# ethanabrooks/hsr-env

Measured on AMD Instinct MI355X. Metric: env-steps/sec (whole node), HSR+1-block, steps_per_action=300, 8192 envs, higher is better.
Workload: dtype f32; 1 GPU; BASELINE config 3: cfg3, all 7 DOFs + 1 block(s), 8192 envs per GPU x 1 GPU(s), steps_per_action=300, geofence=0.05, ctrl~U(ctrlrange) per env-step, done envs reset; envs_per_gpu=8192, global_envs=8192, substeps_per_env_step=300, parallelism=env-shard x1, persistent_kernel=True, hipgraph=False

## Files before the change

hsr_env_amd/csrc/cfg_consts.h:

```cpp
#pragma once
#include "model.h"

struct Kin3_none { static constexpr bool ok = false; };
struct Kin3_cfg1 {
    static constexpr bool ok = true;
    static constexpr int NL = 2, NV = 2, RD0 = 0, NRD = 2, NFREE = 0, F0 = 0;
    static constexpr int parent[2] = {0, 0};
    static constexpr int isfree[2] = {0, 0};
    static constexpr int dofadr[2] = {0, 0};
    static constexpr int dofnum[2] = {0, 2};
    static constexpr int qadr[2] = {0, 0};
    static constexpr int dtype[2] = {0, 0};
    static constexpr int dqadr[2] = {0, 1};
    static constexpr int dlink[2] = {1, 1};
    static constexpr float lpos[2][3] = {{(float)0.0, (float)0.0, (float)0.0}, {(float)-0.46, (float)-0.081, (float)0.0}};
    static constexpr float lmat[2][9] = {{(float)1.0, (float)0.0, (float)0.0, (float)0.0, (float)1.0, (float)0.0, (float)0.0, (float)0.0, (float)1.0}, {(float)1.0, (float)0.0, (float)0.0, (float)0.0, (float)1.0, (float)0.0, (float)0.0, (float)0.0, (float)1.0}};
    static constexpr float lcom[2][3] = {{(float)0.0, (float)0.0, (float)0.0}, {(float)-0.026226165780202215, (float)0.0033597159715531835, (float)0.3351183143878767}};
    static constexpr float linr[2][6] = {{(float)0.0, (float)0.0, (float)0.0, (float)0.0, (float)0.0, (float)0.0}, {(float)17.93115297082212, (float)18.05290570568451, (float)5.361962854382956, (float)-0.18414327285216073, (float)0.6395772498672245, (float)-0.2890701869118962}};
    static constexpr float lmass[2] = {(float)0.0, (float)291.3690145854267};
    static constexpr float daxis[2][3] = {{(float)1.0, (float)0.0, (float)0.0}, {(float)0.0, (float)1.0, (float)0.0}};
    static constexpr float dpos[2][3] = {{(float)0.0, (float)0.0, (float)0.0}, {(float)0.0, (float)0.0, (float)0.0}};
};
static const int kKin3I_cfg1[] = {2, 2, 0, 0, 0, 0, 0, 0, 0, 2, 0, 0, 0, 0, 0, 1, 1, 1};
static const float kKin3F_cfg1[] = {(float)0.0, (float)0.0, (float)0.0, (float)-0.46, (float)-0.081, (float)0.0, (float)1.0, (float)0.0, (float)0.0, (float)0.0, (float)1.0, (float)0.0, (float)0.0, (float)0.0, (float)1.0, (float)1.0, (float)0.0, (float)0.0, (float)0.0, (float)1.0, (float)0.0, (float)0.0, (float)0.0, (float)1.0, (float)0.0, (float)0.0, (float)0.0, (float)-0.026226165780202215, (float)0.0033597159715531835, (float)0.3351183143878767, (float)0.0, (float)0.0, (float)0.0, (float)0.0, (float)0.0, (float)0.0, (float)17.93115297082212, (float)18.05290570568451, (float)5.361962854382956, (float)-0.18414327285216073, (float)0.6395772498672245, (float)-0.2890701869118962, (float)0.0, (float)291.3690145854267, (float)1.0, (float)0.0, (float)0.0, (float)0.0, (float)1.0, (float)0.0, (float)0.0, (float)0.0, (float)0.0, (float)0.0, (float)0.0, (float)0.0};
struct DevModel_cfg1 : DevModel {
    using kin3 = Kin3_cfg1;
    static constexpr int nq = 2, nv = 2, nu = 2, nlink = 2, nbody = 47, ngeom = 17, npair = 30, nslot = 30, nconmax = 16, njmax = 48, nM = 3, ndense = 0, npair_pad = 32, nstatic_geom = 2, nfb = 0, maxdepth = 1, iterations = 100, ls_iterations = 50, mpr_iterations = 50, any_damping = 1, solimp_general = 0, cv_types = 49248;
    static constexpr float timestep = (float)0.002, impratio = (float)2.5, gravz = (float)-9.81, tolerance = (float)1e-08, ls_tolerance = (float)0.01, mpr_tolerance = (float)1e-06, meaninertia = (float)291.3690145854267;
};
struct Kin3_cfg2 {
    static constexpr bool ok = true;
    static constexpr int NL = 3, NV = 8, RD0 = 0, NRD = 2, NFREE = 1, F0 = 2;
    static constexpr int parent[3] = {0, 0, 0};
    static constexpr int isfree[3] = {0, 0, 1};
    static constexpr int dofadr[3] = {0, 0, 2};
    static constexpr int dofnum[3] = {0, 2, 6};
    static constexpr int qadr[3] = {0, 0, 2};
    static constexpr int dtype[8] = {0, 0, 2, 2, 2, 3, 3, 3};
    static constexpr int dqadr[8] = {0, 1, 2, 3, 4, 5, 5, 5};
    static constexpr int dlink[8] = {1, 1, 2, 2, 2, 2, 2, 2};
    static constexpr float lpos[3][3] = {{(float)0.0, (float)0.0, (float)0.0}, {(float)-0.46, (float)-0.081, (float)0.0}, {(float)0.0, (float)0.0, (float)0.422}};
    static constexpr float lmat[3][9] = {{(float)1.0, (float)0.0, (float)0.0, (float)0.0, (float)1.0, (float)0.0, (float)0.0, (float)0.0, (float)1.0}, {(float)1.0, (float)0.0, (float)0.0, (float)0.0, (float)1.0, (float)0.0, (float)0.0, (float)0.0, (float)1.0}, {(float)1.0, (float)0.0, (float)0.0, (float)0.0, (float)1.0, (float)0.0, (float)0.0, (float)0.0, (float)1.0}};
    static constexpr float lcom[3][3] = {{(float)0.0, (float)0.0, (float)0.0}, {(float)-0.026226165780202215, (float)0.0033597159715531835, (float)0.3351183143878767}, {(float)0.0, (float)0.0, (float)0.0}};
    static constexpr float linr[3][6] = {{(float)0.0, (float)0.0, (float)0.0, (float)0.0, (float)0.0, (float)0.0}, {(float)17.93115297082212, (float)18.05290570568451, (float)5.361962854382956, (float)-0.18414327285216073, (float)0.6395772498672245, (float)-0.2890701869118962}, {(float)0.0003046666666666667, (float)0.0009296666666666669, (float)0.0010416666666666669, (float)0.0, (float)0.0, (float)0.0}};
    static constexpr float lmass[3] = {(float)0.0, (float)291.3690145854267, (float)1.0};
    static constexpr float daxis[8][3] = {{(float)1.0, (float)0.0, (float)0.0}, {(float)0.0, (float)1.0, (float)0.0}, {(float)1.0, (float)0.0, (float)0.0}, {(float)0.0, (float)1.0, (float)0.0}, {(float)0.0, (float)0.0, (float)1.0}, {(float)1.0, (float)0.0, (float)0.0}, {(float)0.0, (float)1.0, (float)0.0}, {(float)0.0, (float)0.0, (float)1.0}};
    static constexpr float dpos[8][3] = {{(float)0.0, (float)0.0, (float)0.0}, {(float)0.0, (float)0.0, (float)0.0}, {(float)0.0, (float)0.0, (float)0.0}, {(float)0.0, (float)0.0, (float)0.0}, {(float)0.0, (float)0.0, (float)0.0}, {(float)0.0, (float)0.0, (float)0.0}, {(float)0.0, (float)0.0, (float)0.0}, {(float)0.0, (float)0.0, (float)0.0}};
};
static const int kKin3I_cfg2[] = {3, 8, 0, 0, 0, 0, 0, 1, 0, 0, 2, 0, 2, 6, 0, 0, 2, 0, 0, 2, 2, 2, 3, 3, 3, 0, 1, 2, 3, 4, 5, 5, 5, 1, 1, 2, 2, 2, 2, 2, 2};
static const float kKin3F_cfg2[] = {(float)0.0, (float)0.0, (float)0.0, (float)-0.46, (float)-0.081, (float)0.0, (float)0.0, (float)0.0, (float)0.422, (float)1.0, (float)0.0, (float)0.0, (float)0.0, (float)1.0, (float)0.0, (float)0.0, (float)0.0, (float)1.0, (float)1.0, (float)0.0, (float)0.0, (float)0.0, (float)1.0, (float)0.0, (float)0.0, (float)0.0, (float)1.0, (float)1.0, (float)0.0, (float)0.0, (float)0.0, (float)1.0, (float)0.0, (float)0.0, (float)0.0, (float)1.0, (float)0.0, (float)0.0, (float)0.0, (float)-0.026226165780202215, (float)0.0033597159715531835, (float)0.3351183143878767, (float)0.0, (float)0.0, (float)0.0, (float)0.0, (float)0.0, (float)0.0, (float)0.0, (float)0.0, (float)0.0, (float)17.93115297082212, (float)18.05290570568451, (float)5.361962854382956, (float)-0.18414327285216073, (float)0.6395772498672245, (float)-0.2890701869118962, (float)0.0003046666666666667, (float)0.0009296666666666669, (float)0.0010416666666666669, (float)0.0, (float)0.0, (float)0.0, (float)0.0, (float)291.3690145854267, (float)1.0, (float)1.0, (float)0.0, (float)0.0, (float)0.0, (float)1.0, (float)0.0, (float)1.0, (float)0.0, (float)0.0, (float)0.0, (float)1.0, (float)0.0, (float)0.0, (float)0.0, (float)1.0, (float)1.0, (float)0.0, (float)0.0, (float)0.0, (float)1.0, (float)0.0, (float)0.0, (float)0.0, (float)1.0, (float)0.0, (float)0.0, (float)0.0, (float)0.0, (float)0.0, (float)0.0, (float)0.0, (float)0.0, (float)0.0, (float)0.0, (float)0.0, (float)0.0, (float)0.0, (float)0.0, (float)0.0, (float)0.0, (float)0.0, (float)0.0, (float)0.0, (float)0.0, (float)0.0, (float)0.0, (float)0.0, (float)0.0};
struct DevModel_cfg2 : DevModel {
    using kin3 = Kin3_cfg2;
    static constexpr int nq = 9, nv = 8, nu = 2, nlink = 3, nbody = 48, ngeom = 18, npair = 47, nslot = 57, nconmax = 16, njmax = 48, nM = 36, ndense = 0, npair_pad = 48, nstatic_geom = 2, nfb = 1, maxdepth = 1, iterations = 100, ls_iterations = 50, mpr_iterations = 50, any_damping = 1, solimp_general = 0, cv_types = 49248;
    static constexpr float timestep = (float)0.002, impratio = (float)2.5, gravz = (float)-9.81, tolerance = (float)1e-08, ls_tolerance = (float)0.01, mpr_tolerance = (float)1e-06, meaninertia = (float)73.21753814635669;
};
struct Kin3_cfg3 {
    static constexpr bool ok = true;
    static constexpr int NL = 8, NV = 13, RD0 = 0, NRD = 7, NFREE = 1, F0 = 7;
    static constexpr int parent[8] = {0, 0, 1, 2, 3, 4, 4, 0};
    static constexpr int isfree[8] = {0, 0, 0, 0, 0, 0, 0, 1};
    static constexpr int dofadr[8] = {0, 0, 2, 3, 4, 5, 6, 7};
    static constexpr int dofnum[8] = {0, 2, 1, 1, 1, 1, 1, 6};
    static constexpr int qadr[8] = {0, 0, 2, 3, 4, 5, 6, 7};
    static constexpr int dtype[13] = {0, 0, 0, 1, 1, 1, 1, 2, 2, 2, 3, 3, 3};
    static constexpr int dqadr[13] = {0, 1, 2, 3, 4, 5, 6, 7, 8, 9, 10, 10, 10};
    static constexpr int dlink[13] = {1, 1, 2, 3, 4, 5, 6, 7, 7, 7, 7, 7, 7};
    static constexpr float lpos[8][3] = {{(float)0.0, (float)0.0, (float)0.0}, {(float)-0.46, (float)-0.081, (float)0.0}, {(float)0.0, (float)0.0, (float)0.5}, {(float)0.141, (float)0.078, (float)0.0}, {(float)0.005, (float)0.0, (float)0.345}, {(float)0.02875, (float)0.0245, (float)0.12300000000000001}, {(float)0.02875, (float)-0.0245, (float)0.12300000000000001}, {(float)0.0, (float)0.0, (float)0.422}};
    static constexpr float lmat[8][9] = {{(float)1.0, (float)0.0, (float)0.0, (float)0.0, (float)1.0, (float)0.0, (float)0.0, (float)0.0, (float)1.0}, {(float)1.0, (float)0.0, (float)0.0, (float)0.0, (float)1.0, (float)0.0, (float)0.0, (float)0.0, (float)1.0}, {(float)1.0, (float)0.0, (float)0.0, (float)0.0, (float)1.0, (float)0.0, (float)0.0, (float)0.0, (float)1.0}, {(float)1.0, (float)0.0, (float)0.0, (float)0.0, (float)1.0, (float)0.0, (float)0.0, (float)0.0, (float)1.0}, {(float)-0.3846153846153848, (float)0.0, (float)0.9230769230769234, (float)0.0, (float)1.0, (float)0.0, (float)-0.9230769230769234, (float)0.0, (float)-0.3846153846153848}, {(float)-1.0, (float)0.0, (float)0.0, (float)0.0, (float)-1.0, (float)0.0, (float)0.0, (float)0.0, (float)1.0}, {(float)-1.0, (float)0.0, (float)0.0, (float)0.0, (float)-1.0, (float)0.0, (float)0.0, (float)0.0, (float)1.0}, {(float)1.0, (float)0.0, (float)0.0, (float)0.0, (float)1.0, (float)0.0, (float)0.0, (float)0.0, (float)1.0}};
    static constexpr float lcom[8][3] = {{(float)0.0, (float)0.0, (float)0.0}, {(float)-0.0347552504774637, (float)0.00021983094136669105, (float)0.32107459322514403}, {(float)0.0860739520361204, (float)0.03730696680027092, (float)-0.048237067089018815}, {(float)9.217799537819954e-05, (float)0.005378522674296996, (float)0.16866542736039206}, {(float)-0.0035563457545128956, (float)-4.7945521502316024e-05, (float)0.10077104775564907}, {(float)0.00852311385996903, (float)0.004977974163455939, (float)0.05882302952465269}, {(float)0.008341834250917614, (float)-0.005309505504673415, (float)0.05758153613934645}, {(float)0.0, (float)0.0, (float)0.0}};
    static constexpr float linr[8][6] = {{(float)0.0, (float)0.0, (float)0.0, (float)0.0, (float)0.0, (float)0.0}, {(float)16.250565221699887, (float)15.957245023907413, (float)4.665512029448585, (float)-0.010427084131348163, (float)1.452231512673702, (float)0.008902574260290282}, {(float)0.022820083057640606, (float)0.009954369124611695, (float)0.018401382356491202, (float)-0.0025433386248086133, (float)-0.0016008468094781338, (float)-0.003139446595221039}, {(float)0.09299716849489376, (float)0.08975732788794683, (float)0.009232392506510758, (float)1.6681390623358727e-05, (float)-0.000718335940619342, (float)0.0007228876658435388}, {(float)0.016929615550871812, (float)0.01666906372617751, (float)0.016474889945292476, (float)1.460447612598356e-06, (float)-6.211650900216932e-05, (float)-7.946875319020003e-07}, {(float)0.04612543712881295, (float)0.04613579905249317, (float)0.04510770854929418, (float)-2.5023825011582902e-05, (float)-0.00010925138184770646, (float)-0.00015737797343488998}, {(float)0.046089251928950845, (float)0.04609899116723925, (float)0.04510236718567525, (float)2.5455172651502303e-05, (float)-0.00011036966683664154, (float)0.00016320130800520952}, {(float)0.0003046666666666667, (float)0.0009296666666666669, (float)0.0010416666666666669, (float)0.0, (float)0.0, (float)0.0}};
    static constexpr float lmass[8] = {(float)0.0, (float)277.8610092915329, (float)4.2251095673594845, (float)6.613989657308645, (float)1.482377430363842, (float)0.6047254681827968, (float)0.5818031706792063, (float)1.0};
    static constexpr float daxis[13][3] = {{(float)1.0, (float)0.0, (float)0.0}, {(float)0.0, (float)1.0, (float)0.0}, {(float)0.0, (float)0.0, (float)1.0}, {(float)0.0, (float)-1.0, (float)0.0}, {(float)0.0, (float)0.0, (float)1.0}, {(float)1.0, (float)0.0, (float)0.0}, {(float)-1.0, (float)0.0, (float)0.0}, {(float)1.0, (float)0.0, (float)0.0}, {(float)0.0, (float)1.0, (float)0.0}, {(float)0.0, (float)0.0, (float)1.0}, {(float)1.0, (float)0.0, (float)0.0}, {(float)0.0, (float)1.0, (float)0.0}, {(float)0.0, (float)0.0, (float)1.0}};
    static constexpr float dpos[13][3] = {{(float)0.0, (float)0.0, (float)0.0}, {(float)0.0, (float)0.0, (float)0.0}, {(float)0.0, (float)0.0, (float)0.0}, {(float)0.0, (float)0.0, (float)0.0}, {(float)0.0, (float)0.0, (float)0.0}, {(float)0.0, (float)0.0, (float)0.0}, {(float)0.0, (float)0.0, (float)0.0}, {(float)0.0, (float)0.0, (float)0.0}, {(float)0.0, (float)0.0, (float)0.0}, {(float)0.0, (float)0.0, (float)0.0}, {(float)0.0, (float)0.0, (float)0.0}, {(float)0.0, (float)0.0, (float)0.0}, {(float)0.0, (float)0.0, (float)0.0}};
};
static const int kKin3I_cfg3[] = {8, 13, 0, 0, 1, 2, 3, 4, 4, 0, 0, 0, 0, 0, 0, 0, 0, 1, 0, 0, 2, 3, 4, 5, 6, 7, 0, 2, 1, 1, 1, 1, 1, 6, 0, 0, 2, 3, 4, 5, 6, 7, 0, 0, 0, 1, 1, 1, 1, 2, 2, 2, 3, 3, 3, 0, 1, 2, 3, 4, 5, 6, 7, 8, 9, 10, 10, 10, 1, 1, 2, 3, 4, 5, 6, 7, 7, 7, 7, 7, 7};
static const float kKin3F_cfg3[] = {(float)0.0, (float)0.0, (float)0.0, (float)-0.46, (float)-0.081, (float)0.0, (float)0.0, (float)0.0, (float)0.5, (float)0.141, (float)0.078, (float)0.0, (float)0.005, (float)0.0, (float)0.345, (float)0.02875, (float)0.0245, (float)0.12300000000000001, (float)0.02875, (float)-0.0245, (float)0.12300000000000001, (float)0.0, (float)0.0, (float)0.422, (float)1.0, (float)0.0, (float)0.0, (float)0.0, (float)1.0, (float)0.0, (float)0.0, (float)0.0, (float)1.0, (float)1.0, (float)0.0, (float)0.0, (float)0.0, (float)1.0, (float)0.0, (float)0.0, (float)0.0, (float)1.0, (float)1.0, (float)0.0, (float)0.0, (float)0.0, (float)1.0, (float)0.0, (float)0.0, (float)0.0, (float)1.0, (float)1.0, (float)0.0, (float)0.0, (float)0.0, (float)1.0, (float)0.0, (float)0.0, (float)0.0, (float)1.0, (float)-0.3846153846153848, (float)0.0, (float)0.9230769230769234, (float)0.0, (float)1.0, (float)0.0, (float)-0.9230769230769234, (float)0.0, (float)-0.3846153846153848, (float)-1.0, (float)0.0, (float)0.0, (float)0.0, (float)-1.0, (float)0.0, (float)0.0, (float)0.0, (float)1.0, (float)-1.0, (float)0.0, (float)0.0, (float)0.0, (float)-1.0, (float)0.0, (float)0.0, (float)0.0, (float)1.0, (float)1.0, (float)0.0, (float)0.0, (float)0.0, (float)1.0, (float)0.0, (float)0.0, (float)0.0, (float)1.0, (float)0.0, (float)0.0, (float)0.0, (float)-0.0347552504774637, (float)0.00021983094136669105, (float)0.32107459322514403, (float)0.0860739520361204, (float)0.03730696680027092, (float)-0.048237067089018815, (float)9.217799537819954e-05, (float)0.005378522674296996, (float)0.16866542736039206, (float)-0.0035563457545128956, (float)-4.7945521502316024e-05, (float)0.10077104775564907, (float)0.00852311385996903, (float)0.004977974163455939, (float)0.05882302952465269, (float)0.008341834250917614, (float)-0.005309505504673415, (float)0.05758153613934645, (float)0.0, (float)0.0, (float)0.0, (float)0.0, (float)0.0, (float)0.0, (float)0.0, (float)0.0, (float)0.0, (float)16.250565221699887, (float)15.957245023907413, (float)4.665512029448585, (float)-0.010427084131348163, (float)1.452231512673702, (float)0.008902574260290282, (float)0.022820083057640606, (float)0.009954369124611695, (float)0.018401382356491202, (float)-0.0025433386248086133, (float)-0.0016008468094781338, (float)-0.003139446595221039, (float)0.09299716849489376, (float)0.08975732788794683, (float)0.009232392506510758, (float)1.6681390623358727e-05, (float)-0.000718335940619342, (float)0.0007228876658435388, (float)0.016929615550871812, (float)0.01666906372617751, (float)0.016474889945292476, (float)1.460447612598356e-06, (float)-6.211650900216932e-05, (float)-7.946875319020003e-07, (float)0.04612543712881295, (float)0.04613579905249317, (float)0.04510770854929418, (float)-2.5023825011582902e-05, (float)-0.00010925138184770646, (float)-0.00015737797343488998, (float)0.046089251928950845, (float)0.04609899116723925, (float)0.04510236718567525, (float)2.5455172651502303e-05, (float)-0.00011036966683664154, (float)0.00016320130800520952, (float)0.0003046666666666667, (float)0.0009296666666666669, (float)0.0010416666666666669, (float)0.0, (float)0.0, (float)0.0, (float)0.0, (float)277.8610092915329, (float)4.2251095673594845, (float)6.613989657308645, (float)1.482377430363842, (float)0.6047254681827968, (float)0.5818031706792063, (float)1.0, (float)1.0, (float)0.0, (float)0.0, (float)0.0, (float)1.0, (float)0.0, (float)0.0, (float)0.0, (float)1.0, (float)0.0, (float)-1.0, (float)0.0, (float)0.0, (float)0.0, (float)1.0, (float)1.0, (float)0.0, (float)0.0, (float)-1.0, (float)0.0, (float)0.0, (float)1.0, (float)0.0, (float)0.0, (float)0.0, (float)1.0, (float)0.0, (float)0.0, (float)0.0, (float)1.0, (float)1.0, (float)0.0, (float)0.0, (float)0.0, (float)1.0, (float)0.0, (float)0.0, (float)0.0, (float)1.0, (float)0.0, (float)0.0, (float)0.0, (float)0.0, (float)0.0, (float)0.0, (float)0.0, (float)0.0, (float)0.0, (float)0.0, (float)0.0, (float)0.0, (float)0.0, (float)0.0, (float)0.0, (float)0.0, (float)0.0, (float)0.0, (float)0.0, (float)0.0, (float)0.0, (float)0.0, (float)0.0, (float)0.0, (float)0.0, (float)0.0, (float)0.0, (float)0.0, (float)0.0, (float)0.0, (float)0.0, (float)0.0, (float)0.0, (float)0.0, (float)0.0, (float)0.0, (float)0.0, (float)0.0, (float)0.0};
struct DevModel_cfg3 : DevModel {
    using kin3 = Kin3_cfg3;
    static constexpr int nq = 14, nv = 13, nu = 7, nlink = 8, nbody = 48, ngeom = 18, npair = 114, nslot = 124, nconmax = 16, njmax = 48, nM = 91, ndense = 7, npair_pad = 120, nstatic_geom = 2, nfb = 1, maxdepth = 5, iterations = 100, ls_iterations = 50, mpr_iterations = 50, any_damping = 1, solimp_general = 0, cv_types = 49376;
    static constexpr float timestep = (float)0.002, impratio = (float)2.5, gravz = (float)-9.81, tolerance = (float)1e-08, ls_tolerance = (float)0.01, mpr_tolerance = (float)1e-06, meaninertia = (float)46.161990948437406;
};
struct Kin3_cfg4 {
    static constexpr bool ok = true;
    static constexpr int NL = 10, NV = 25, RD0 = 0, NRD = 7, NFREE = 3, F0 = 7;
    static constexpr int parent[10] = {0, 0, 1, 2, 3, 4, 4, 0, 0, 0};
    static constexpr int isfree[10] = {0, 0, 0, 0, 0, 0, 0, 1, 1, 1};
    static constexpr int dofadr[10] = {0, 0, 2, 3, 4, 5, 6, 7, 13, 19};
    static constexpr int dofnum[10] = {0, 2, 1, 1, 1, 1, 1, 6, 6, 6};
    static constexpr int qadr[10] = {0, 0, 2, 3, 4, 5, 6, 7, 14, 21};
    static constexpr int dtype[25] = {0, 0, 0, 1, 1, 1, 1, 2, 2, 2, 3, 3, 3, 2, 2, 2, 3, 3, 3, 2, 2, 2, 3, 3, 3};
    static constexpr int dqadr[25] = {0, 1, 2, 3, 4, 5, 6, 7, 8, 9, 10, 10, 10, 14, 15, 16, 17, 17, 17, 21, 22, 23, 24, 24, 24};
    static constexpr int dlink[25] = {1, 1, 2, 3, 4, 5, 6, 7, 7, 7, 7, 7, 7, 8, 8, 8, 8, 8, 8, 9, 9, 9, 9, 9, 9};
    static constexpr float lpos[10][3] = {{(float)0.0, (float)0.0, (float)0.0}, {(float)-0.46, (float)-0.081, (float)0.0}, {(float)0.0, (float)0.0, (float)0.5}, {(float)0.141, (float)0.078, (float)0.0}, {(float)0.005, (float)0.0, (float)0.345}, {(float)0.02875, (float)0.0245, (float)0.12300000000000001}, {(float)0.02875, (float)-0.0245, (float)0.12300000000000001}, {(float)0.0, (float)-0.12, (float)0.422}, {(float)0.0, (float)0.0, (float)0.422}, {(float)0.0, (float)0.12, (float)0.422}};
    static constexpr float lmat[10][9] = {{(float)1.0, (float)0.0, (float)0.0, (float)0.0, (float)1.0, (float)0.0, (float)0.0, (float)0.0, (float)1.0}, {(float)1.0, (float)0.0, (float)0.0, (float)0.0, (float)1.0, (float)0.0, (float)0.0, (float)0.0, (float)1.0}, {(float)1.0, (float)0.0, (float)0.0, (float)0.0, (float)1.0, (float)0.0, (float)0.0, (float)0.0, (float)1.0}, {(float)1.0, (float)0.0, (float)0.0, (float)0.0, (float)1.0, (float)0.0, (float)0.0, (float)0.0, (float)1.0}, {(float)-0.3846153846153848, (float)0.0, (float)0.9230769230769234, (float)0.0, (float)1.0, (float)0.0, (float)-0.9230769230769234, (float)0.0, (float)-0.3846153846153848}, {(float)-1.0, (float)0.0, (float)0.0, (float)0.0, (float)-1.0, (float)0.0, (float)0.0, (float)0.0, (float)1.0}, {(float)-1.0, (float)0.0, (float)0.0, (float)0.0, (float)-1.0, (float)0.0, (float)0.0, (float)0.0, (float)1.0}, {(float)1.0, (float)0.0, (float)0.0, (float)0.0, (float)1.0, (float)0.0, (float)0.0, (float)0.0, (float)1.0}, {(float)1.0, (float)0.0, (float)0.0, (float)0.0, (float)1.0, (float)0.0, (float)0.0, (float)0.0, (float)1.0}, {(float)1.0, (float)0.0, (float)0.0, (float)0.0, (float)1.0, (float)0.0, (float)0.0, (float)0.0, (float)1.0}};
    static constexpr float lcom[10][3] = {{(float)0.0, (float)0.0, (float)0.0}, {(float)-0.0347552504774637, (float)0.00021983094136669105, (float)0.32107459322514403}, {(float)0.0860739520361204, (float)0.03730696680027092, (float)-0.048237067089018815}, {(float)9.217799537819954e-05, (float)0.005378522674296996, (float)0.16866542736039206}, {(float)-0.0035563457545128956, (float)-4.7945521502316024e-05, (float)0.10077104775564907}, {(float)0.00852311385996903, (float)0.004977974163455939, (float)0.05882302952465269}, {(float)0.008341834250917614, (float)-0.005309505504673415, (float)0.05758153613934645}, {(float)0.0, (float)0.0, (float)0.0}, {(float)0.0, (float)0.0, (float)0.0}, {(float)0.0, (float)0.0, (float)0.0}};
    static constexpr float linr[10][6] = {{(float)0.0, (float)0.0, (float)0.0, (float)0.0, (float)0.0, (float)0.0}, {(float)16.250565221699887, (float)15.957245023907413, (float)4.665512029448585, (float)-0.010427084131348163, (float)1.452231512673702, (float)0.008902574260290282}, {(float)0.022820083057640606, (float)0.009954369124611695, (float)0.018401382356491202, (float)-0.0025433386248086133, (float)-0.0016008468094781338, (float)-0.003139446595221039}, {(float)0.09299716849489376, (float)0.08975732788794683, (float)0.009232392506510758, (float)1.6681390623358727e-05, (float)-0.000718335940619342, (float)0.0007228876658435388}, {(float)0.016929615550871812, (float)0.01666906372617751, (float)0.016474889945292476, (float)1.460447612598356e-06, (float)-6.211650900216932e-05, (float)-7.946875319020003e-07}, {(float)0.04612543712881295, (float)0.04613579905249317, (float)0.04510770854929418, (float)-2.5023825011582902e-05, (float)-0.00010925138184770646, (float)-0.00015737797343488998}, {(float)0.046089251928950845, (float)0.04609899116723925, (float)0.04510236718567525, (float)2.5455172651502303e-05, (float)-0.00011036966683664154, (float)0.00016320130800520952}, {(float)0.0003046666666666667, (float)0.0009296666666666669, (float)0.0010416666666666669, (float)0.0, (float)0.0, (float)0.0}, {(float)0.0003046666666666667, (float)0.0009296666666666669, (float)0.0010416666666666669, (float)0.0, (float)0.0, (float)0.0}, {(float)0.0003046666666666667, (float)0.0009296666666666669, (float)0.0010416666666666669, (float)0.0, (float)0.0, (float)0.0}};
    static constexpr float lmass[10] = {(float)0.0, (float)277.8610092915329, (float)4.2251095673594845, (float)6.613989657308645, (float)1.482377430363842, (float)0.6047254681827968, (float)0.5818031706792063, (float)1.0, (float)1.0, (float)1.0};
    static constexpr float daxis[25][3] = {{(float)1.0, (float)0.0, (float)0.0}, {(float)0.0, (float)1.0, (float)0.0}, {(float)0.0, (float)0.0, (float)1.0}, {(float)0.0, (float)-1.0, (float)0.0}, {(float)0.0, (float)0.0, (float)1.0}, {(float)1.0, (float)0.0, (float)0.0}, {(float)-1.0, (float)0.0, (float)0.0}, {(float)1.0, (float)0.0, (float)0.0}, {(float)0.0, (float)1.0, (float)0.0}, {(float)0.0, (float)0.0, (float)1.0}, {(float)1.0, (float)0.0, (float)0.0}, {(float)0.0, (float)1.0, (float)0.0}, {(float)0.0, (float)0.0, (float)1.0}, {(float)1.0, (float)0.0, (float)0.0}, {(float)0.0, (float)1.0, (float)0.0}, {(float)0.0, (float)0.0, (float)1.0}, {(float)1.0, (float)0.0, (float)0.0}, {(float)0.0, (float)1.0, (float)0.0}, {(float)0.0, (float)0.0, (float)1.0}, {(float)1.0, (float)0.0, (float)0.0}, {(float)0.0, (float)1.0, (float)0.0}, {(float)0.0, (float)0.0, (float)1.0}, {(float)1.0, (float)0.0, (float)0.0}, {(float)0.0, (float)1.0, (float)0.0}, {(float)0.0, (float)0.0, (float)1.0}};
    static constexpr float dpos[25][3] = {{(float)0.0, (float)0.0, (float)0.0}, {(float)0.0, (float)0.0, (float)0.0}, {(float)0.0, (float)0.0, (float)0.0}, {(float)0.0, (float)0.0, (float)0.0}, {(float)0.0, (float)0.0, (float)0.0}, {(float)0.0, (float)0.0, (float)0.0}, {(float)0.0, (float)0.0, (float)0.0}, {(float)0.0, (float)0.0, (float)0.0}, {(float)0.0, (float)0.0, (float)0.0}, {(float)0.0, (float)0.0, (float)0.0}, {(float)0.0, (float)0.0, (float)0.0}, {(float)0.0, (float)0.0, (float)0.0}, {(float)0.0, (float)0.0, (float)0.0}, {(float)0.0, (float)0.0, (float)0.0}, {(float)0.0, (float)0.0, (float)0.0}, {(float)0.0, (float)0.0, (float)0.0}, {(float)0.0, (float)0.0, (float)0.0}, {(float)0.0, (float)0.0, (float)0.0}, {(float)0.0, (float)0.0, (float)0.0}, {(float)0.0, (float)0.0, (float)0.0}, {(float)0.0, (float)0.0, (float)0.0}, {(float)0.0, (float)0.0, (float)0.0}, {(float)0.0, (float)0.0, (float)0.0}, {(float)0.0, (float)0.0, (float)0.0}, {(float)0.0, (float)0.0, (float)0.0}};
};
static const int kKin3I_cfg4[] = {10, 25, 0, 0, 1, 2, 3, 4, 4, 0, 0, 0, 0, 0, 0, 0, 0, 0, 0, 1, 1, 1, 0, 0, 2, 3, 4, 5, 6, 7, 13, 19, 0, 2, 1, 1, 1, 1, 1, 6, 6, 6, 0, 0, 2, 3, 4, 5, 6, 7, 14, 21, 0, 0, 0, 1, 1, 1, 1, 2, 2, 2, 3, 3, 3, 2, 2, 2, 3, 3, 3, 2, 2, 2, 3, 3, 3, 0, 1, 2, 3, 4, 5, 6, 7, 8, 9, 10, 10, 10, 14, 15, 16, 17, 17, 17, 21, 22, 23, 24, 24, 24, 1, 1, 2, 3, 4, 5, 6, 7, 7, 7, 7, 7, 7, 8, 8, 8, 8, 8, 8, 9, 9, 9, 9, 9, 9};
static const float kKin3F_cfg4[] = {(float)0.0, (float)0.0, (float)0.0, (float)-0.46, (float)-0.081, (float)0.0, (float)0.0, (float)0.0, (float)0.5, (float)0.141, (float)0.078, (float)0.0, (float)0.005, (float)0.0, (float)0.345, (float)0.02875, (float)0.0245, (float)0.12300000000000001, (float)0.02875, (float)-0.0245, (float)0.12300000000000001, (float)0.0, (float)-0.12, (float)0.422, (float)0.0, (float)0.0, (float)0.422, (float)0.0, (float)0.12, (float)0.422, (float)1.0, (float)0.0, (float)0.0, (float)0.0, (float)1.0, (float)0.0, (float)0.0, (float)0.0, (float)1.0, (float)1.0, (float)0.0, (float)0.0, (float)0.0, (float)1.0, (float)0.0, (float)0.0, (float)0.0, (float)1.0, (float)1.0, (float)0.0, (float)0.0, (float)0.0, (float)1.0, (float)0.0, (float)0.0, (float)0.0, (float)1.0, (float)1.0, (float)0.0, (float)0.0, (float)0.0, (float)1.0, (float)0.0, (float)0.0, (float)0.0, (float)1.0, (float)-0.3846153846153848, (float)0.0, (float)0.9230769230769234, (float)0.0, (float)1.0, (float)0.0, (float)-0.9230769230769234, (float)0.0, (float)-0.3846153846153848, (float)-1.0, (float)0.0, (float)0.0, (float)0.0, (float)-1.0, (float)0.0, (float)0.0, (float)0.0, (float)1.0, (float)-1.0, (float)0.0, (float)0.0, (float)0.0, (float)-1.0, (float)0.0, (float)0.0, (float)0.0, (float)1.0, (float)1.0, (float)0.0, (float)0.0, (float)0.0, (float)1.0, (float)0.0, (float)0.0, (float)0.0, (float)1.0, (float)1.0, (float)0.0, (float)0.0, (float)0.0, (float)1.0, (float)0.0, (float)0.0, (float)0.0, (float)1.0, (float)1.0, (float)0.0, (float)0.0, (float)0.0, (float)1.0, (float)0.0, (float)0.0, (float)0.0, (float)1.0, (float)0.0, (float)0.0, (float)0.0, (float)-0.0347552504774637, (float)0.00021983094136669105, (float)0.32107459322514403, (float)0.0860739520361204, (float)0.03730696680027092, (float)-0.048237067089018815, (float)9.217799537819954e-05, (float)0.005378522674296996, (float)0.16866542736039206, (float)-0.0035563457545128956, (float)-4.7945521502316024e-05, (float)0.10077104775564907, (float)0.00852311385996903, (float)0.004977974163455939, (float)0.05882302952465269, (float)0.008341834250917614, (float)-0.005309505504673415, (float)0.05758153613934645, (float)0.0, (float)0.0, (float)0.0, (float)0.0, (float)0.0, (float)0.0, (float)0.0, (float)0.0, (float)0.0, (float)0.0, (float)0.0, (float)0.0, (float)0.0, (float)0.0, (float)0.0, (float)16.250565221699887, (float)15.957245023907413, (float)4.665512029448585, (float)-0.010427084131348163, (float)1.452231512673702, (float)0.008902574260290282, (float)0.022820083057640606, (float)0.009954369124611695, (float)0.018401382356491202, (float)-0.0025433386248086133, (float)-0.0016008468094781338, (float)-0.003139446595221039, (float)0.09299716849489376, (float)0.08975732788794683, (float)0.009232392506510758, (float)1.6681390623358727e-05, (float)-0.000718335940619342, (float)0.0007228876658435388, (float)0.016929615550871812, (float)0.01666906372617751, (float)0.016474889945292476, (float)1.460447612598356e-06, (float)-6.211650900216932e-05, (float)-7.946875319020003e-07, (float)0.04612543712881295, (float)0.04613579905249317, (float)0.04510770854929418, (float)-2.5023825011582902e-05, (float)-0.00010925138184770646, (float)-0.00015737797343488998, (float)0.046089251928950845, (float)0.04609899116723925, (float)0.04510236718567525, (float)2.5455172651502303e-05, (float)-0.00011036966683664154, (float)0.00016320130800520952, (float)0.0003046666666666667, (float)0.0009296666666666669, (float)0.0010416666666666669, (float)0.0, (float)0.0, (float)0.0, (float)0.0003046666666666667, (float)0.0009296666666666669, (float)0.0010416666666666669, (float)0.0, (float)0.0, (float)0.0, (float)0.0003046666666666667, (float)0.0009296666666666669, (float)0.0010416666666666669, (float)0.0, (float)0.0, (float)0.0, (float)0.0, (float)277.8610092915329, (float)4.2251095673594845, (float)6.613989657308645, (float)1.482377430363842, (float)0.6047254681827968, (float)0.5818031706792063, (float)1.0, (float)1.0, (float)1.0, (float)1.0, (float)0.0, (float)0.0, (float)0.0, (float)1.0, (float)0.0, (float)0.0, (float)0.0, (float)1.0, (float)0.0, (float)-1.0, (float)0.0, (float)0.0, (float)0.0, (float)1.0, (float)1.0, (float)0.0, (float)0.0, (float)-1.0, (float)0.0, (float)0.0, (float)1.0, (float)0.0, (float)0.0, (float)0.0, (float)1.0, (float)0.0, (float)0.0, (float)0.0, (float)1.0, (float)1.0, (float)0.0, (float)0.0, (float)0.0, (float)1.0, (float)0.0, (float)0.0, (float)0.0, (float)1.0, (float)1.0, (float)0.0, (float)0.0, (float)0.0, (float)1.0, (float)0.0, (float)0.0, (float)0.0, (float)1.0, (float)1.0, (float)0.0, (float)0.0, (float)0.0, (float)1.0, (float)0.0, (float)0.0, (float)0.0, (float)1.0, (float)1.0, (float)0.0, (float)0.0, (float)0.0, (float)1.0, (float)0.0, (float)0.0, (float)0.0, (float)1.0, (float)1.0, (float)0.0, (float)0.0, (float)0.0, (float)1.0, (float)0.0, (float)0.0, (float)0.0, (float)1.0, (float)0.0, (float)0.0, (float)0.0, (float)0.0, (float)0.0, (float)0.0, (float)0.0, (float)0.0, (float)0.0, (float)0.0, (float)0.0, (float)0.0, (float)0.0, (float)0.0, (float)0.0, (float)0.0, (float)0.0, (float)0.0, (float)0.0, (float)0.0, (float)0.0, (float)0.0, (float)0.0, (float)0.0, (float)0.0, (float)0.0, (float)0.0, (float)0.0, (float)0.0, (float)0.0, (float)0.0, (float)0.0, (float)0.0, (float)0.0, (float)0.0, (float)0.0, (float)0.0, (float)0.0, (float)0.0, (float)0.0, (float)0.0, (float)0.0, (float)0.0, (float)0.0, (float)0.0, (float)0.0, (float)0.0, (float)0.0, (float)0.0, (float)0.0, (float)0.0, (float)0.0, (float)0.0, (float)0.0, (float)0.0, (float)0.0, (float)0.0, (float)0.0, (float)0.0, (float)0.0, (float)0.0, (float)0.0, (float)0.0, (float)0.0, (float)0.0, (float)0.0, (float)0.0, (float)0.0, (float)0.0, (float)0.0, (float)0.0, (float)0.0, (float)0.0, (float)0.0, (float)0.0};
struct DevModel_cfg4 : DevModel {
    using kin3 = Kin3_cfg4;
    static constexpr int nq = 28, nv = 25, nu = 7, nlink = 10, nbody = 50, ngeom = 20, npair = 151, nslot = 202, nconmax = 32, njmax = 124, nM = 325, ndense = 7, npair_pad = 152, nstatic_geom = 2, nfb = 3, maxdepth = 5, iterations = 100, ls_iterations = 50, mpr_iterations = 50, any_damping = 1, solimp_general = 0, cv_types = 49376;
    static constexpr float timestep = (float)0.002, impratio = (float)2.5, gravz = (float)-9.81, tolerance = (float)1e-08, ls_tolerance = (float)0.01, mpr_tolerance = (float)1e-06, meaninertia = (float)24.244417373187453;
};
struct Kin3_cupboard {
    static constexpr bool ok = true;
    static constexpr int NL = 8, NV = 13, RD0 = 6, NRD = 7, NFREE = 1, F0 = 1;
    static constexpr int parent[8] = {0, 0, 0, 2, 3, 4, 5, 5};
    static constexpr int isfree[8] = {0, 1, 0, 0, 0, 0, 0, 0};
    static constexpr int dofadr[8] = {0, 0, 6, 8, 9, 10, 11, 12};
    static constexpr int dofnum[8] = {0, 6, 2, 1, 1, 1, 1, 1};
    static constexpr int qadr[8] = {0, 0, 7, 9, 10, 11, 12, 13};
    static constexpr int dtype[13] = {2, 2, 2, 3, 3, 3, 0, 0, 0, 1, 1, 1, 1};
    static constexpr int dqadr[13] = {0, 1, 2, 3, 3, 3, 7, 8, 9, 10, 11, 12, 13};
    static constexpr int dlink[13] = {1, 1, 1, 1, 1, 1, 2, 2, 3, 4, 5, 6, 7};
    static constexpr float lpos[8][3] = {{(float)0.0, (float)0.0, (float)0.0}, {(float)-0.1, (float)0.0, (float)0.418}, {(float)-0.46, (float)-0.081, (float)0.0}, {(float)0.0, (float)0.0, (float)0.5}, {(float)0.141, (float)0.078, (float)0.0}, {(float)0.005, (float)0.0, (float)0.345}, {(float)0.02875, (float)0.0245, (float)0.12300000000000001}, {(float)0.02875, (float)-0.0245, (float)0.12300000000000001}};
    static constexpr float lmat[8][9] = {{(float)1.0, (float)0.0, (float)0.0, (float)0.0, (float)1.0, (float)0.0, (float)0.0, (float)0.0, (float)1.0}, {(float)1.0, (float)0.0, (float)0.0, (float)0.0, (float)1.0, (float)0.0, (float)0.0, (float)0.0, (float)1.0}, {(float)1.0, (float)0.0, (float)0.0, (float)0.0, (float)1.0, (float)0.0, (float)0.0, (float)0.0, (float)1.0}, {(float)1.0, (float)0.0, (float)0.0, (float)0.0, (float)1.0, (float)0.0, (float)0.0, (float)0.0, (float)1.0}, {(float)1.0, (float)0.0, (float)0.0, (float)0.0, (float)1.0, (float)0.0, (float)0.0, (float)0.0, (float)1.0}, {(float)-0.3846153846153848, (float)0.0, (float)0.9230769230769234, (float)0.0, (float)1.0, (float)0.0, (float)-0.9230769230769234, (float)0.0, (float)-0.3846153846153848}, {(float)-1.0, (float)0.0, (float)0.0, (float)0.0, (float)-1.0, (float)0.0, (float)0.0, (float)0.0, (float)1.0}, {(float)-1.0, (float)0.0, (float)0.0, (float)0.0, (float)-1.0, (float)0.0, (float)0.0, (float)0.0, (float)1.0}};
    static constexpr float lcom[8][3] = {{(float)0.0, (float)0.0, (float)0.0}, {(float)0.0, (float)0.0, (float)0.0}, {(float)-0.0347552504774637, (float)0.00021983094136669105, (float)0.32107459322514403}, {(float)0.0860739520361204, (float)0.03730696680027092, (float)-0.048237067089018815}, {(float)9.217799537819954e-05, (float)0.005378522674296996, (float)0.16866542736039206}, {(float)-0.0035563457545128956, (float)-4.7945521502316024e-05, (float)0.10077104775564907}, {(float)0.00852311385996903, (float)0.004977974163455939, (float)0.05882302952465269}, {(float)0.008341834250917614, (float)-0.005309505504673415, (float)0.05758153613934645}};
    static constexpr float linr[8][6] = {{(float)0.0, (float)0.0, (float)0.0, (float)0.0, (float)0.0, (float)0.0}, {(float)0.0003046666666666667, (float)0.0009296666666666669, (float)0.0010416666666666669, (float)0.0, (float)0.0, (float)0.0}, {(float)16.250565221699887, (float)15.957245023907413, (float)4.665512029448585, (float)-0.010427084131348163, (float)1.452231512673702, (float)0.008902574260290282}, {(float)0.022820083057640606, (float)0.009954369124611695, (float)0.018401382356491202, (float)-0.0025433386248086133, (float)-0.0016008468094781338, (float)-0.003139446595221039}, {(float)0.09299716849489376, (float)0.08975732788794683, (float)0.009232392506510758, (float)1.6681390623358727e-05, (float)-0.000718335940619342, (float)0.0007228876658435388}, {(float)0.016929615550871812, (float)0.01666906372617751, (float)0.016474889945292476, (float)1.460447612598356e-06, (float)-6.211650900216932e-05, (float)-7.946875319020003e-07}, {(float)0.04612543712881295, (float)0.04613579905249317, (float)0.04510770854929418, (float)-2.5023825011582902e-05, (float)-0.00010925138184770646, (float)-0.00015737797343488998}, {(float)0.046089251928950845, (float)0.04609899116723925, (float)0.04510236718567525, (float)2.5455172651502303e-05, (float)-0.00011036966683664154, (float)0.00016320130800520952}};
    static constexpr float lmass[8] = {(float)0.0, (float)1.0, (float)277.8610092915329, (float)4.2251095673594845, (float)6.613989657308645, (float)1.482377430363842, (float)0.6047254681827968, (float)0.5818031706792063};
    static constexpr float daxis[13][3] = {{(float)1.0, (float)0.0, (float)0.0}, {(float)0.0, (float)1.0, (float)0.0}, {(float)0.0, (float)0.0, (float)1.0}, {(float)1.0, (float)0.0, (float)0.0}, {(float)0.0, (float)1.0, (float)0.0}, {(float)0.0, (float)0.0, (float)1.0}, {(float)1.0, (float)0.0, (float)0.0}, {(float)0.0, (float)1.0, (float)0.0}, {(float)0.0, (float)0.0, (float)1.0}, {(float)0.0, (float)-1.0, (float)0.0}, {(float)0.0, (float)0.0, (float)1.0}, {(float)1.0, (float)0.0, (float)0.0}, {(float)-1.0, (float)0.0, (float)0.0}};
    static constexpr float dpos[13][3] = {{(float)0.0, (float)0.0, (float)0.0}, {(float)0.0, (float)0.0, (float)0.0}, {(float)0.0, (float)0.0, (float)0.0}, {(float)0.0, (float)0.0, (float)0.0}, {(float)0.0, (float)0.0, (float)0.0}, {(float)0.0, (float)0.0, (float)0.0}, {(float)0.0, (float)0.0, (float)0.0}, {(float)0.0, (float)0.0, (float)0.0}, {(float)0.0, (float)0.0, (float)0.0}, {(float)0.0, (float)0.0, (float)0.0}, {(float)0.0, (float)0.0, (float)0.0}, {(float)0.0, (float)0.0, (float)0.0}, {(float)0.0, (float)0.0, (float)0.0}};
};
static const int kKin3I_cupboard[] = {8, 13, 0, 0, 0, 2, 3, 4, 5, 5, 0, 1, 0, 0, 0, 0, 0, 0, 0, 0, 6, 8, 9, 10, 11, 12, 0, 6, 2, 1, 1, 1, 1, 1, 0, 0, 7, 9, 10, 11, 12, 13, 2, 2, 2, 3, 3, 3, 0, 0, 0, 1, 1, 1, 1, 0, 1, 2, 3, 3, 3, 7, 8, 9, 10, 11, 12, 13, 1, 1, 1, 1, 1, 1, 2, 2, 3, 4, 5, 6, 7};
static const float kKin3F_cupboard[] = {(float)0.0, (float)0.0, (float)0.0, (float)-0.1, (float)0.0, (float)0.418, (float)-0.46, (float)-0.081, (float)0.0, (float)0.0, (float)0.0, (float)0.5, (float)0.141, (float)0.078, (float)0.0, (float)0.005, (float)0.0, (float)0.345, (float)0.02875, (float)0.0245, (float)0.12300000000000001, (float)0.02875, (float)-0.0245, (float)0.12300000000000001, (float)1.0, (float)0.0, (float)0.0, (float)0.0, (float)1.0, (float)0.0, (float)0.0, (float)0.0, (float)1.0, (float)1.0, (float)0.0, (float)0.0, (float)0.0, (float)1.0, (float)0.0, (float)0.0, (float)0.0, (float)1.0, (float)1.0, (float)0.0, (float)0.0, (float)0.0, (float)1.0, (float)0.0, (float)0.0, (float)0.0, (float)1.0, (float)1.0, (float)0.0, (float)0.0, (float)0.0, (float)1.0, (float)0.0, (float)0.0, (float)0.0, (float)1.0, (float)1.0, (float)0.0, (float)0.0, (float)0.0, (float)1.0, (float)0.0, (float)0.0, (float)0.0, (float)1.0, (float)-0.3846153846153848, (float)0.0, (float)0.9230769230769234, (float)0.0, (float)1.0, (float)0.0, (float)-0.9230769230769234, (float)0.0, (float)-0.3846153846153848, (float)-1.0, (float)0.0, (float)0.0, (float)0.0, (float)-1.0, (float)0.0, (float)0.0, (float)0.0, (float)1.0, (float)-1.0, (float)0.0, (float)0.0, (float)0.0, (float)-1.0, (float)0.0, (float)0.0, (float)0.0, (float)1.0, (float)0.0, (float)0.0, (float)0.0, (float)0.0, (float)0.0, (float)0.0, (float)-0.0347552504774637, (float)0.00021983094136669105, (float)0.32107459322514403, (float)0.0860739520361204, (float)0.03730696680027092, (float)-0.048237067089018815, (float)9.217799537819954e-05, (float)0.005378522674296996, (float)0.16866542736039206, (float)-0.0035563457545128956, (float)-4.7945521502316024e-05, (float)0.10077104775564907, (float)0.00852311385996903, (float)0.004977974163455939, (float)0.05882302952465269, (float)0.008341834250917614, (float)-0.005309505504673415, (float)0.05758153613934645, (float)0.0, (float)0.0, (float)0.0, (float)0.0, (float)0.0, (float)0.0, (float)0.0003046666666666667, (float)0.0009296666666666669, (float)0.0010416666666666669, (float)0.0, (float)0.0, (float)0.0, (float)16.250565221699887, (float)15.957245023907413, (float)4.665512029448585, (float)-0.010427084131348163, (float)1.452231512673702, (float)0.008902574260290282, (float)0.022820083057640606, (float)0.009954369124611695, (float)0.018401382356491202, (float)-0.0025433386248086133, (float)-0.0016008468094781338, (float)-0.003139446595221039, (float)0.09299716849489376, (float)0.08975732788794683, (float)0.009232392506510758, (float)1.6681390623358727e-05, (float)-0.000718335940619342, (float)0.0007228876658435388, (float)0.016929615550871812, (float)0.01666906372617751, (float)0.016474889945292476, (float)1.460447612598356e-06, (float)-6.211650900216932e-05, (float)-7.946875319020003e-07, (float)0.04612543712881295, (float)0.04613579905249317, (float)0.04510770854929418, (float)-2.5023825011582902e-05, (float)-0.00010925138184770646, (float)-0.00015737797343488998, (float)0.046089251928950845, (float)0.04609899116723925, (float)0.04510236718567525, (float)2.5455172651502303e-05, (float)-0.00011036966683664154, (float)0.00016320130800520952, (float)0.0, (float)1.0, (float)277.8610092915329, (float)4.2251095673594845, (float)6.613989657308645, (float)1.482377430363842, (float)0.6047254681827968, (float)0.5818031706792063, (float)1.0, (float)0.0, (float)0.0, (float)0.0, (float)1.0, (float)0.0, (float)0.0, (float)0.0, (float)1.0, (float)1.0, (float)0.0, (float)0.0, (float)0.0, (float)1.0, (float)0.0, (float)0.0, (float)0.0, (float)1.0, (float)1.0, (float)0.0, (float)0.0, (float)0.0, (float)1.0, (float)0.0, (float)0.0, (float)0.0, (float)1.0, (float)0.0, (float)-1.0, (float)0.0, (float)0.0, (float)0.0, (float)1.0, (float)1.0, (float)0.0, (float)0.0, (float)-1.0, (float)0.0, (float)0.0, (float)0.0, (float)0.0, (float)0.0, (float)0.0, (float)0.0, (float)0.0, (float)0.0, (float)0.0, (float)0.0, (float)0.0, (float)0.0, (float)0.0, (float)0.0, (float)0.0, (float)0.0, (float)0.0, (float)0.0, (float)0.0, (float)0.0, (float)0.0, (float)0.0, (float)0.0, (float)0.0, (float)0.0, (float)0.0, (float)0.0, (float)0.0, (float)0.0, (float)0.0, (float)0.0, (float)0.0, (float)0.0, (float)0.0, (float)0.0, (float)0.0, (float)0.0, (float)0.0, (float)0.0, (float)0.0};
struct DevModel_cupboard : DevModel {
    using kin3 = Kin3_cupboard;
    static constexpr int nq = 14, nv = 13, nu = 7, nlink = 8, nbody = 53, ngeom = 28, npair = 274, nslot = 354, nconmax = 16, njmax = 48, nM = 91, ndense = 13, npair_pad = 280, nstatic_geom = 12, nfb = 0, maxdepth = 5, iterations = 100, ls_iterations = 50, mpr_iterations = 50, any_damping = 1, solimp_general = 0, cv_types = 49376;
    static constexpr float timestep = (float)0.002, impratio = (float)2.5, gravz = (float)-9.81, tolerance = (float)1e-08, ls_tolerance = (float)0.01, mpr_tolerance = (float)1e-06, meaninertia = (float)46.161990948437406;
};

struct CfgConstRow { const char *name; int i[22]; float f[7]; };
static const CfgConstRow kCfgConsts[] = {
    {"cfg1", {2, 2, 2, 2, 47, 17, 30, 30, 16, 48, 3, 0, 32, 2, 0, 1, 100, 50, 50, 1, 0, 49248}, {(float)0.002, (float)2.5, (float)-9.81, (float)1e-08, (float)0.01, (float)1e-06, (float)291.3690145854267}},
    {"cfg2", {9, 8, 2, 3, 48, 18, 47, 57, 16, 48, 36, 0, 48, 2, 1, 1, 100, 50, 50, 1, 0, 49248}, {(float)0.002, (float)2.5, (float)-9.81, (float)1e-08, (float)0.01, (float)1e-06, (float)73.21753814635669}},
    {"cfg3", {14, 13, 7, 8, 48, 18, 114, 124, 16, 48, 91, 7, 120, 2, 1, 5, 100, 50, 50, 1, 0, 49376}, {(float)0.002, (float)2.5, (float)-9.81, (float)1e-08, (float)0.01, (float)1e-06, (float)46.161990948437406}},
    {"cfg4", {28, 25, 7, 10, 50, 20, 151, 202, 32, 124, 325, 7, 152, 2, 3, 5, 100, 50, 50, 1, 0, 49376}, {(float)0.002, (float)2.5, (float)-9.81, (float)1e-08, (float)0.01, (float)1e-06, (float)24.244417373187453}},
    {"cupboard", {14, 13, 7, 8, 53, 28, 274, 354, 16, 48, 91, 13, 280, 12, 0, 5, 100, 50, 50, 1, 0, 49376}, {(float)0.002, (float)2.5, (float)-9.81, (float)1e-08, (float)0.01, (float)1e-06, (float)46.161990948437406}},
};
struct Kin3Check { const int *i; int ni; const float *f; int nf; };
static const Kin3Check kKin3Checks[] = {{kKin3I_cfg1, (int)(sizeof kKin3I_cfg1 / sizeof(int)), kKin3F_cfg1, (int)(sizeof kKin3F_cfg1 / sizeof(float))}, {kKin3I_cfg2, (int)(sizeof kKin3I_cfg2 / sizeof(int)), kKin3F_cfg2, (int)(sizeof kKin3F_cfg2 / sizeof(float))}, {kKin3I_cfg3, (int)(sizeof kKin3I_cfg3 / sizeof(int)), kKin3F_cfg3, (int)(sizeof kKin3F_cfg3 / sizeof(float))}, {kKin3I_cfg4, (int)(sizeof kKin3I_cfg4 / sizeof(int)), kKin3F_cfg4, (int)(sizeof kKin3F_cfg4 / sizeof(float))}, {kKin3I_cupboard, (int)(sizeof kKin3I_cupboard / sizeof(int)), kKin3F_cupboard, (int)(sizeof kKin3F_cupboard / sizeof(float))}};
static inline void cfg_const_values(const DevModel &d, int *i, float *f) {
    const int iv[] = {d.nq, d.nv, d.nu, d.nlink, d.nbody, d.ngeom, d.npair, d.nslot, d.nconmax, d.njmax, d.nM, d.ndense, d.npair_pad, d.nstatic_geom, d.nfb, d.maxdepth, d.iterations, d.ls_iterations, d.mpr_iterations, d.any_damping, d.solimp_general, d.cv_types};
    const float fv[] = {d.timestep, d.impratio, d.gravz, d.tolerance, d.ls_tolerance, d.mpr_tolerance, d.meaninertia};
    for (int k = 0; k < 22; k++) i[k] = iv[k];
    for (int k = 0; k < 7; k++) f[k] = fv[k];
}
```

hsr_env_amd/csrc/collide.h:

```cpp
#pragma once
#include "devmath.h"
#include "model.h"

struct KinGlobal {
    const DevModel &m;
    __device__ __forceinline__ int link_dofadr(int l) const { return m.link_dofadr[l]; }
    __device__ __forceinline__ int link_dofnum(int l) const { return m.link_dofnum[l]; }
    __device__ __forceinline__ int link_free(int l) const { return m.link_free[l]; }
    __device__ __forceinline__ int link_qposadr(int l) const { return m.link_qposadr[l]; }
    __device__ __forceinline__ int link_parent(int l) const { return m.link_parent[l]; }
    __device__ __forceinline__ v3 link_pos(int l) const { return ld3(m.link_pos, l); }
    __device__ __forceinline__ m3 link_mat(int l) const { return ldm(m.link_mat, l); }
    __device__ __forceinline__ v3 link_com(int l) const { return ld3(m.link_com, l); }
    __device__ __forceinline__ float link_mass(int l) const { return m.link_mass[l]; }
    __device__ __forceinline__ void link_inertia(int l, float *o) const {
#pragma unroll
        for (int i = 0; i < 6; i++) o[i] = m.link_inertia[6 * l + i]; }
    __device__ __forceinline__ int dof_qposadr(int k) const { return m.dof_qposadr[k]; }
    __device__ __forceinline__ int dof_type(int k) const { return m.dof_type[k]; }
    __device__ __forceinline__ v3 dof_axis(int k) const { return ld3(m.dof_axis, k); }
    __device__ __forceinline__ v3 dof_pos(int k) const { return ld3(m.dof_pos, k); }
};
__device__ __forceinline__ v3 sel3(bool c, v3 a, v3 b) { return mk3(c ? a.x : b.x, c ? a.y : b.y, c ? a.z : b.z); }

// ... 53 lines not shown
}

template <class KC>
__device__ __forceinline__ void kin_link_dyn(const KC &K, float gravz, int l, View qvel, View xpos, View xmat, View ang, View lin, View anc, View ld,
                                             View lw, View lvo, View lal, View lao) {
    const int d0 = K.link_dofadr(l);
    const m3 R = xmat.getm(l);
    const v3 xl = xpos.get3(l);
    v3 w, vo, al, ao;
    if (K.link_free(l)) {
        vo = mk3(qvel[d0], qvel[d0 + 1], qvel[d0 + 2]);
        w = mulmv(R, mk3(qvel[d0 + 3], qvel[d0 + 4], qvel[d0 + 5]));
        al = mk3(0, 0, 0); ao = mk3(0, 0, 0);
    } else {
        const int p = K.link_parent(l);
        const v3 wp = lw.get3(p), vop = lvo.get3(p), alp = lal.get3(p), aop = lao.get3(p);
        const v3 r = xl - xpos.get3(p);
        w = wp; al = alp;
        vo = vop + cross(wp, r);
        ao = aop + cross(alp, r) + cross(wp, cross(wp, r));
        for (int k = d0; k < d0 + K.link_dofnum(l); k++) {
            const float qd = qvel[k];
            if (K.dof_type(k) == DOF_SLIDE) {
                const v3 sx = lin.get3(k);
                vo = vo + sx * qd;
                ao = ao + cross(wp, sx) * (2 * qd);
            } else {
                const v3 a = ang.get3(k);
                const v3 rho = xl - anc.get3(k), rc = r - rho;
                const v3 wl = w + a * qd, all = al + cross(w, a) * qd;
                const v3 ac = aop + cross(alp, rc) + cross(wp, cross(wp, rc));
                const v3 vc = vop + cross(wp, rc);
                ao = ac + cross(all, rho) + cross(wl, cross(wl, rho));
                vo = vc + cross(wl, rho);
                w = wl; al = all;
            }
        }
    }
    lw.set3(l, w); lvo.set3(l, vo); lal.set3(l, al); lao.set3(l, ao);
    float li[6];
    K.link_inertia(l, li);
    m3 Il, Rt;
    Il.a[0] = li[0]; Il.a[1] = li[3]; Il.a[2] = li[4]; Il.a[3] = li[3]; Il.a[4] = li[1]; Il.a[5] = li[5]; Il.a[6] = li[4]; Il.a[7] = li[5]; Il.a[8] = li[2];
#pragma unroll
    for (int i = 0; i < 3; i++)
#pragma unroll
        for (int j = 0; j < 3; j++) Rt.a[3 * i + j] = R.a[3 * j + i];
    const m3 I = mulmm(mulmm(R, Il), Rt);
    const v3 com = xl + mulmv(R, K.link_com(l)), rc = com - xl;
    const v3 acom = ao + cross(al, rc) + cross(w, cross(w, rc));
    const v3 F = (acom - mk3(0, 0, gravz)) * K.link_mass(l);
    const v3 Nt = mulmv(I, al) + cross(w, mulmv(I, w));
    const int b = 15 * l;
    ld[b] = com.x; ld[b + 1] = com.y; ld[b + 2] = com.z;
    ld[b + 3] = I.a[0]; ld[b + 4] = I.a[4]; ld[b + 5] = I.a[8]; ld[b + 6] = I.a[1]; ld[b + 7] = I.a[2]; ld[b + 8] = I.a[5];
    ld[b + 9] = F.x; ld[b + 10] = F.y; ld[b + 11] = F.z; ld[b + 12] = Nt.x; ld[b + 13] = Nt.y; ld[b + 14] = Nt.z;
}

__device__ __forceinline__ void kin_link0(View xpos, View xmat, View ld, View lw, View lvo, View lal, View lao) {
    m3 I;
#pragma unroll
    for (int k = 0; k < 9; k++) I.a[k] = (k % 4 == 0) ? 1.f : 0.f;
    xpos.set3(0, mk3(0, 0, 0));
    xmat.setm(0, I);
    lw.set3(0, mk3(0, 0, 0)); lvo.set3(0, mk3(0, 0, 0)); lal.set3(0, mk3(0, 0, 0)); lao.set3(0, mk3(0, 0, 0));
    for (int k = 0; k < 15; k++) ld[k] = 0;
}

__device__ void kin_env(const DevModel &m, View qpos, View qvel, View xpos, View xmat, View ang, View lin, View anc, View ld,
                        View lw, View lvo, View lal, View lao) {
    kin_link0(xpos, xmat, ld, lw, lvo, lal, lao);
    const KinGlobal K{m};
    for (int l = 1; l < m.nlink; l++) kin_link_pose(K, l, qpos, xpos, xmat, ang, lin, anc);
    for (int l = 1; l < m.nlink; l++) kin_link_dyn(K, m.gravz, l, qvel, xpos, xmat, ang, lin, anc, ld, lw, lvo, lal, lao);
}

__global__ void __launch_bounds__(64) k_kinematics(DevModel m, DevState s) {
    extern __shared__ float ktile[];
    if (blockIdx.x == 0) for (int i = threadIdx.x; i < m.npair_pad; i += 64) s.pair_count[i] = 0;
    const int e_raw = blockIdx.x * 64 + threadIdx.x;
    const bool live = e_raw < s.N && !s.done[e_raw < s.N ? e_raw : 0];
    const int e = live ? e_raw : 0;
    const int N = s.N, TS = s.kstride + 24 * m.nlink + 1;
    float *tl = ktile + threadIdx.x * TS;
    if (live) {
    View qpos{s.qpos + e, N}, xpos{tl + s.kstride, 1}, xmat{tl + s.kstride + 3 * m.nlink, 1};
    View ang{tl, 1}, lin{tl + 3 * m.nv, 1}, anc{tl + 6 * m.nv, 1};
    View qvel{s.qvel + e, N}, ld{tl + 9 * m.nv, 1};
    View lw{tl + s.kstride + 12 * m.nlink, 1}, lvo{tl + s.kstride + 15 * m.nlink, 1}, lal{tl + s.kstride + 18 * m.nlink, 1}, lao{tl + s.kstride + 21 * m.nlink, 1};
    kin_env(m, qpos, qvel, xpos, xmat, ang, lin, anc, ld, lw, lvo, lal, lao);
    for (int i = 9 * m.nv + 15 * m.nlink; i < s.kstride; i++) tl[i] = 0.f;
    }
    __syncthreads();
    const int e0 = blockIdx.x * 64, KS = s.kstride;
    const unsigned long long livemask = __ballot(live);
    for (int le = 0; le < 64; le++) {
        if (!((livemask >> le) & 1ull)) continue;
        float *dst = s.kin_aos + (size_t)(e0 + le) * KS;
        const float *src = ktile + le * TS;
        for (int i = threadIdx.x; i < KS; i += 64) dst[i] = src[i];
    }
    if (live) {
        for (int i = 0; i < 3 * m.nlink; i++) s.xpos[(size_t)i * N + e] = tl[s.kstride + i];
        for (int i = 0; i < 9 * m.nlink; i++) s.xmat[(size_t)i * N + e] = tl[s.kstride + 3 * m.nlink + i];
        for (int i = 0; i < 6 * m.nlink; i++) s.lvel[(size_t)i * N + e] = tl[s.kstride + 12 * m.nlink + i];
    }
}

struct Geom {
    int type, nvert;
    v3 pos, size;
    v3 bc, bh;
    m3 mat;
    const float4 *verts;
};

__device__ __forceinline__ Geom load_geom_v(const DevModel &m, View xpos, View xmat, int g);
__device__ __forceinline__ Geom load_geom(const DevModel &m, const DevState &s, int g, int e) {
    return load_geom_v(m, View{s.xpos + e, s.N}, View{s.xmat + e, s.N}, g);
}
__device__ __forceinline__ Geom load_geom_v(const DevModel &m, View xpos, View xmat, int g) {
    Geom G;
    const int l = m.geom_link[g];
    const m3 R = xmat.getm(l);
    G.pos = xpos.get3(l) + mulmv(R, ld3(m.geom_pos, g));
    G.mat = mulmm(R, ldm(m.geom_mat, g));
    G.type = m.geom_type[g];
    G.size = ld3(m.geom_size, g);
    G.bc = G.pos + mulmv(G.mat, mk3(m.geom_aabb[6 * g], m.geom_aabb[6 * g + 1], m.geom_aabb[6 * g + 2]));
    G.bh = mk3(m.geom_aabb[6 * g + 3], m.geom_aabb[6 * g + 4], m.geom_aabb[6 * g + 5]);
    G.verts = nullptr;
    G.nvert = m.geom_meshnum[g];
    return G;
}

enum { VID_BITS = 12, VID_NONE = (1 << VID_BITS) - 1 };
template <int W> __device__ __forceinline__ void sup_merge(float &b, int &idx, float pb, int pi) {
    const bool take = (pb > b) | ((pb == b) & (pi < idx));
    b = take ? pb : b; idx = take ? pi : idx;
}
__device__ __forceinline__ v3 support_vertex(const Geom &G, int vid) {
    v3 loc;
    if (G.type == GEOM_BOX) loc = mk3((vid & 1) ? G.size.x : -G.size.x, (vid & 2) ? G.size.y : -G.size.y, (vid & 4) ? G.size.z : -G.size.z);
    else { const float4 w = G.verts[vid]; loc = mk3(w.x, w.y, w.z); }
    return mulmv(G.mat, loc) + G.pos;
}
enum { GEOM_TYPES_ANY = 0xff };
template <int TM, int T> __device__ __forceinline__ bool geom_type_is(int type) {
    if constexpr (((TM >> T) & 1) == 0) return false;
    else return type == T;
}
template <class T, class = void> struct ConvexTypes { static constexpr int first = GEOM_TYPES_ANY, second = GEOM_TYPES_ANY; };
template <class T> struct ConvexTypes<T, std::enable_if_t<!std::is_same<T, DevModel>::value>> { static constexpr int first = T::cv_types & 0xff, second = (T::cv_types >> 8) & 0xff; };
template <int W = 1, int TM = GEOM_TYPES_ANY> __device__ __forceinline__ v3 support(const Geom &G, v3 dir, int *vid = nullptr) {
    const v3 dl = mulmtv(G.mat, dir);
    v3 loc;
    if (vid) *vid = VID_NONE;
    if (geom_type_is<TM, GEOM_BOX>(G.type)) {
        loc = mk3(dl.x > 0 ? G.size.x : -G.size.x, dl.y > 0 ? G.size.y : -G.size.y, dl.z > 0 ? G.size.z : -G.size.z);
        if (vid) *vid = (dl.x > 0 ? 1 : 0) | (dl.y > 0 ? 2 : 0) | (dl.z > 0 ? 4 : 0);
    } else if (geom_type_is<TM, GEOM_CYLINDER>(G.type)) {
        const float r2 = dl.x * dl.x + dl.y * dl.y, ir = frsq(r2);
        if (r2 > HSR_MINVAL * HSR_MINVAL) { loc.x = dl.x * ir * G.size.x; loc.y = dl.y * ir * G.size.x; } else { loc.x = 0; loc.y = 0; }
        loc.z = dl.z > 0 ? G.size.y : -G.size.y;
    } else if (geom_type_is<TM, GEOM_SPHERE>(G.type)) {
        loc = normalized(dl) * G.size.x;
    } else {
      if constexpr (W > 1) {
        const int sub = threadIdx.x & (W - 1);
        float b = -3.0e38f;
        int idx = 0x7fffffff;
        const float *gverts = (const float *)G.verts;
        auto gvert = [&](int i) { return make_float4(gverts[4 * i], gverts[4 * i + 1], gverts[4 * i + 2], 0.f); };
        for (int i0 = 0; i0 < G.nvert; i0 += 4 * W) {
            float4 q[4];
            int ic[4];
#pragma unroll
            for (int u = 0; u < 4; u++) { const int i = i0 + u * W + sub; ic[u] = i < G.nvert ? i : 0; q[u] = gvert(ic[u]); }
#pragma unroll
            for (int u = 0; u < 4; u++) {
                const float t = q[u].x * dl.x + q[u].y * dl.y + q[u].z * dl.z;
                if (t > b) { b = t; idx = ic[u]; }
            }
        }
        sup_merge<W>(b, idx, __builtin_bit_cast(float, __builtin_amdgcn_update_dpp(0, __builtin_bit_cast(int, b), 0xB1, 0xf, 0xf, true)), __builtin_amdgcn_update_dpp(0, idx, 0xB1, 0xf, 0xf, true));
        if constexpr (W >= 4) sup_merge<W>(b, idx, __builtin_bit_cast(float, __builtin_amdgcn_update_dpp(0, __builtin_bit_cast(int, b), 0x4E, 0xf, 0xf, true)), __builtin_amdgcn_update_dpp(0, idx, 0x4E, 0xf, 0xf, true));
        if constexpr (W >= 8) sup_merge<W>(b, idx, __builtin_bit_cast(float, __builtin_amdgcn_update_dpp(0, __builtin_bit_cast(int, b), 0x141, 0xf, 0xf, true)), __builtin_amdgcn_update_dpp(0, idx, 0x141, 0xf, 0xf, true));
        if constexpr (W >= 16) sup_merge<W>(b, idx, __builtin_bit_cast(float, __builtin_amdgcn_update_dpp(0, __builtin_bit_cast(int, b), 0x140, 0xf, 0xf, true)), __builtin_amdgcn_update_dpp(0, idx, 0x140, 0xf, 0xf, true));
        const float4 w = gvert(G.nvert > 0 ? idx : 0);
        loc = mk3(w.x, w.y, w.z);
        if (vid) *vid = G.nvert > 0 ? idx : 0;
      } else {
        float bA = -3.0e38f, bB = -3.0e38f;
        int iA = 0, iB = 1;
        int i = 0;
        for (; i + 8 <= G.nvert; i += 8) {
            float4 q[8];
#pragma unroll
            for (int u = 0; u < 8; u++) q[u] = G.verts[i + u];
#pragma unroll
            for (int u = 0; u < 8; u += 2) {
                const float ta = q[u].x * dl.x + q[u].y * dl.y + q[u].z * dl.z, tb = q[u + 1].x * dl.x + q[u + 1].y * dl.y + q[u + 1].z * dl.z;
                iA = ta > bA ? i + u : iA; bA = fmaxf(bA, ta);
                iB = tb > bB ? i + u + 1 : iB; bB = fmaxf(bB, tb);
            }
        }
        for (; i < G.nvert; i++) {
            const float4 a = G.verts[i];
            const float t = a.x * dl.x + a.y * dl.y + a.z * dl.z;
            if (i & 1) { iB = t > bB ? i : iB; bB = fmaxf(bB, t); } else { iA = t > bA ? i : iA; bA = fmaxf(bA, t); }
        }
        const int best = (bB > bA || (bB == bA && iB < iA)) ? iB : iA;
        const float4 w = G.verts[G.nvert > 0 ? best : 0];
        loc = mk3(w.x, w.y, w.z);
        if (vid) *vid = G.nvert > 0 ? best : 0;
      }
    }
    return mulmv(G.mat, loc) + G.pos;
}

struct ContactOut {
    float *con;
    int slot, cnt, maxcnt;
    __device__ __forceinline__ void add(v3 pos, v3 n, float dist) {
        if (cnt >= maxcnt) return;
        float4 *r = reinterpret_cast<float4 *>(con + (size_t)(slot + cnt) * 8);
        r[0] = make_float4(pos.x, pos.y, pos.z, n.x);
        r[1] = make_float4(n.y, n.z, dist, 0.f);
        cnt++;
    }
};

__device__ __forceinline__ void collide_plane_box(const Geom &P, const Geom &B, ContactOut &out) {
    const v3 n = col(P.mat, 2);
#pragma unroll
    for (int i = 0; i < 8; i++) {
        const v3 loc = mk3((i & 1) ? B.size.x : -B.size.x, (i & 2) ? B.size.y : -B.size.y, (i & 4) ? B.size.z : -B.size.z);
        const v3 c = mulmv(B.mat, loc) + B.pos;
        const float dist = dot(c - P.pos, n);
        if (dist < 0 && out.cnt < 4) out.add(c - n * (0.5f * dist), n, dist);
    }
}

__device__ __forceinline__ void collide_plane_convex(const Geom &P, const Geom &Cx, ContactOut &out) {
    const v3 n = col(P.mat, 2);
    const v3 p = support(Cx, -n);
    const float dist = dot(p - P.pos, n);
    if (!(dist < 0)) return;
    out.add(p - n * (0.5f * dist), n, dist);
    if (out.maxcnt <= 1) return;
    v3 t1 = (n.y > -0.5f && n.y < 0.5f) ? mk3(0, 1, 0) : mk3(0, 0, 1);
    t1 = normalized(t1 - n * dot(n, t1));
    const v3 t2 = cross(n, t1);
    v3 kept[4];
    kept[0] = p;
    int nk = 1;
    const float cs[3][2] = {{1.f, 0.f}, {-0.5f, 0.8660254f}, {-0.5f, -0.8660254f}};
#pragma unroll
    for (int i = 0; i < 3; i++) {
        if (nk >= out.maxcnt) break;
        const v3 q = support(Cx, (t1 * cs[i][0] + t2 * cs[i][1]) * 0.1f - n);
        const float dq = dot(q - P.pos, n);
        bool take = dq < 0;
#pragma unroll
        for (int j = 0; j < 4; j++) if (j < nk) { const v3 e = q - kept[j]; take = take && !(dot(e, e) < 1e-10f); }
        if (take) {
            out.add(q - n * (0.5f * dq), n, dq);
#pragma unroll
            for (int j = 1; j < 4; j++) if (j == nk) kept[j] = q;
            nk++;
        }
    }
}

#define POLY(buf, i, k) poly[(((buf) * 8 + (i)) * 3 + (k)) * pstride + poff]
__device__ __forceinline__ int clip_poly(float *poly, int pstride, int poff, int src, int n, v3 axis, float lim, v3 origin) {
    const int dst = src ^ 1;
    int no = 0;
    for (int i = 0; i < n; i++) {
        const int i2 = (i + 1 == n) ? 0 : i + 1;
        const v3 a = mk3(POLY(src, i, 0), POLY(src, i, 1), POLY(src, i, 2));
        const v3 b = mk3(POLY(src, i2, 0), POLY(src, i2, 1), POLY(src, i2, 2));
        const float da = dot(a - origin, axis) - lim, db = dot(b - origin, axis) - lim;
        if (da <= 0 && no < 8) { POLY(dst, no, 0) = a.x; POLY(dst, no, 1) = a.y; POLY(dst, no, 2) = a.z; no++; }
        if (((da < 0 && db > 0) || (da > 0 && db < 0)) && no < 8) {
            const float t = da * frcp(da - db);
            POLY(dst, no, 0) = a.x + t * (b.x - a.x); POLY(dst, no, 1) = a.y + t * (b.y - a.y); POLY(dst, no, 2) = a.z + t * (b.z - a.z);
            no++;
        }
    }
    return no;
}

__device__ __forceinline__ void collide_box_box_p(const Geom &G1, const Geom &G2, ContactOut &out, float *poly, int pstride, int poff) {
    v3 A[3], B[3];
    float s1[3] = {G1.size.x, G1.size.y, G1.size.z}, s2[3] = {G2.size.x, G2.size.y, G2.size.z};
#pragma unroll
    for (int i = 0; i < 3; i++) { A[i] = col(G1.mat, i); B[i] = col(G2.mat, i); }
    const v3 dv = G2.pos - G1.pos;
    float C[3][3], aC[3][3];
#pragma unroll
    for (int i = 0; i < 3; i++)
#pragma unroll
        for (int j = 0; j < 3; j++) { C[i][j] = dot(A[i], B[j]); aC[i][j] = fabsf(C[i][j]); }
    float best = -3.0e38f;
    int code = -1;
    v3 bestn = mk3(0, 0, 0);
    bool sepfound = false;
#pragma unroll
    for (int i = 0; i < 3; i++) {
        const float t = dot(dv, A[i]);
        const float sep = fabsf(t) - (s1[i] + s2[0] * aC[i][0] + s2[1] * aC[i][1] + s2[2] * aC[i][2]);
        if (sep > 0) sepfound = true;
        if (sep > best) { best = sep; code = i; bestn = A[i] * (t < 0 ? -1.f : 1.f); }
    }
#pragma unroll
    for (int j = 0; j < 3; j++) {
        const float t = dot(dv, B[j]);
        const float sep = fabsf(t) - (s2[j] + s1[0] * aC[0][j] + s1[1] * aC[1][j] + s1[2] * aC[2][j]);
        if (sep > 0) sepfound = true;
        if (sep > best) { best = sep; code = 3 + j; bestn = B[j] * (t < 0 ? -1.f : 1.f); }
    }
    if (sepfound) return;
#pragma unroll
    for (int i = 0; i < 3; i++)
#pragma unroll
        for (int j = 0; j < 3; j++) {
            v3 L = cross(A[i], B[j]);
            const float ln = norm(L);
            if (ln < 1e-6f) continue;
            L = L * frcp(ln);
            const float t = dot(dv, L);
            float ra = 0, rb = 0;
#pragma unroll
            for (int k = 0; k < 3; k++) { ra += s1[k] * fabsf(dot(A[k], L)); rb += s2[k] * fabsf(dot(B[k], L)); }
            const float sep = fabsf(t) - (ra + rb);
            if (sep > 0) sepfound = true;
            if (sep * 1.05f > best + 1e-9f) { best = sep; code = 6 + 3 * i + j; bestn = L * (t < 0 ? -1.f : 1.f); }
        }
    if (sepfound) return;
    if (code < 6) {
        const bool ref1 = code < 3;
        const int ax = ref1 ? code : code - 3;
        const v3 pr = ref1 ? G1.pos : G2.pos, pi = ref1 ? G2.pos : G1.pos;
        v3 Ar[3], Ai[3];
        float sr[3], si[3];
#pragma unroll
        for (int k = 0; k < 3; k++) { Ar[k] = ref1 ? A[k] : B[k]; Ai[k] = ref1 ? B[k] : A[k]; sr[k] = ref1 ? s1[k] : s2[k]; si[k] = ref1 ? s2[k] : s1[k]; }
        const v3 nref = bestn * (ref1 ? 1.f : -1.f);
        int jx = 0;
        float bd = -1.f;
#pragma unroll
        for (int j = 0; j < 3; j++) { const float t = fabsf(dot(nref, Ai[j])); if (t > bd) { bd = t; jx = j; } }
        const v3 Aj = jx == 0 ? Ai[0] : (jx == 1 ? Ai[1] : Ai[2]);
        const v3 Aj1 = jx == 0 ? Ai[1] : (jx == 1 ? Ai[2] : Ai[0]);
        const v3 Aj2 = jx == 0 ? Ai[2] : (jx == 1 ? Ai[0] : Ai[1]);
        const float sj = jx == 0 ? si[0] : (jx == 1 ? si[1] : si[2]);
        const float sj1 = jx == 0 ? si[1] : (jx == 1 ? si[2] : si[0]);
        const float sj2 = jx == 0 ? si[2] : (jx == 1 ? si[0] : si[1]);
        const float sgn = dot(nref, Aj) > 0 ? -1.f : 1.f;
        const v3 fc = pi + Aj * (sgn * sj);
        const float sg[4][2] = {{1, 1}, {-1, 1}, {-1, -1}, {1, -1}};
#pragma unroll
        for (int k = 0; k < 4; k++) {
            const v3 v = fc + Aj1 * (sg[k][0] * sj1) + Aj2 * (sg[k][1] * sj2);
            POLY(0, k, 0) = v.x; POLY(0, k, 1) = v.y; POLY(0, k, 2) = v.z;
        }
        const v3 Au = ax == 0 ? Ar[1] : (ax == 1 ? Ar[2] : Ar[0]);
        const v3 Av = ax == 0 ? Ar[2] : (ax == 1 ? Ar[0] : Ar[1]);
        const float su = ax == 0 ? sr[1] : (ax == 1 ? sr[2] : sr[0]);
        const float sv = ax == 0 ? sr[2] : (ax == 1 ? sr[0] : sr[1]);
        const float sa = ax == 0 ? sr[0] : (ax == 1 ? sr[1] : sr[2]);
        int np = 4, buf = 0;
        np = clip_poly(poly, pstride, poff, buf, np, Au, su, pr); buf ^= 1;
        if (np) { np = clip_poly(poly, pstride, poff, buf, np, -Au, su, pr); buf ^= 1; }
        if (np) { np = clip_poly(poly, pstride, poff, buf, np, Av, sv, pr); buf ^= 1; }
        if (np) { np = clip_poly(poly, pstride, poff, buf, np, -Av, sv, pr); buf ^= 1; }
        for (int k = 0; k < np; k++) {
            const v3 v = mk3(POLY(buf, k, 0), POLY(buf, k, 1), POLY(buf, k, 2));
            const float dist = dot(v - pr, nref) - sa;
            if (dist < 0) out.add(v - nref * (0.5f * dist), bestn, dist);
        }
    } else {
        const int i = (code - 6) / 3, j = (code - 6) % 3;
        v3 pa = G1.pos, pb = G2.pos;
#pragma unroll
        for (int k = 0; k < 3; k++) {
            if (k != i) pa = pa + A[k] * ((dot(bestn, A[k]) > 0 ? 1.f : -1.f) * s1[k]);
            if (k != j) pb = pb + B[k] * ((dot(bestn, B[k]) > 0 ? -1.f : 1.f) * s2[k]);
        }
        const v3 Ai_ = i == 0 ? A[0] : (i == 1 ? A[1] : A[2]);
        const v3 Bj_ = j == 0 ? B[0] : (j == 1 ? B[1] : B[2]);
        const v3 w = pa - pb;
        const float b = dot(Ai_, Bj_), dd = dot(Ai_, w), ee = dot(Bj_, w), den = 1.f - b * b;
        const float t = den > 1e-12f ? (b * ee - dd) / den : 0.f, uu = den > 1e-12f ? (ee - b * dd) / den : 0.f;
        const v3 qa = pa + Ai_ * t, qb = pb + Bj_ * uu;
        out.add((qa + qb) * 0.5f, bestn, best);
    }
}
#undef POLY
__device__ __forceinline__ void collide_box_box(const Geom &G1, const Geom &G2, ContactOut &out, float *poly, int lane) { collide_box_box_p(G1, G2, out, poly, 64, lane); }

__device__ __forceinline__ v3 shfl3_8(v3 a, int src) { return mk3(__shfl(a.x, src, 8), __shfl(a.y, src, 8), __shfl(a.z, src, 8)); }
template <int CTRL> __device__ __forceinline__ int dppi_(int v) { return __builtin_amdgcn_update_dpp(0, v, CTRL, 0xf, 0xf, true); }
template <int CTRL> __device__ __forceinline__ float dppf_(float v) { return __builtin_bit_cast(float, dppi_<CTRL>(__builtin_bit_cast(int, v))); }
template <int Q> __device__ __forceinline__ int sg8_bcast(int v) { const int lo = dppi_<0x150 + Q>(v), hi = dppi_<0x158 + Q>(v); return (threadIdx.x & 8) ? hi : lo; }
template <int Q> __device__ __forceinline__ float sg8_bcast(float v) { return __builtin_bit_cast(float, sg8_bcast<Q>(__builtin_bit_cast(int, v))); }
__device__ __forceinline__ float sg8_next(float v) { return dppf_<0x101>(v); }
struct NoStamp { __device__ __forceinline__ void operator()(int) const {} };
template <class ST = NoStamp> __device__ __forceinline__ int collide_box_box_w8(const Geom &G1, const Geom &G2, float *con, int slot, int maxcnt, float *scr, ST stamp = ST()) {
    const int sub = threadIdx.x & 7;
    v3 A[3], B[3];
    float s1[3] = {G1.size.x, G1.size.y, G1.size.z}, s2[3] = {G2.size.x, G2.size.y, G2.size.z};
#pragma unroll
// ... 458 lines not shown
```

hsr_env_amd/csrc/host_create.h:

```cpp

static void read_switches(hsr_batch *b) {
    auto env = [](const char *name) { const char *v = getenv(name); return v ? v : ""; };
    auto is0 = [&](const char *name) { return strcmp(env(name), "0") == 0; };
    auto set = [&](const char *name) { return getenv(name) != nullptr; };
    b->sw.no_const = set("HSR_NO_CONST") && !is0("HSR_NO_CONST");
    if (set("HSR_NFB")) b->sw.nfb_max = std::max(atoi(env("HSR_NFB")), 0);
    b->sw.tables_lds = is0("HSR_TABLES_GLOBAL");
    b->sw.debug = set("HSR_DEBUG");
    if (set("HSR_SOLO")) b->solo_servers = atoi(env("HSR_SOLO"));
    if (atof(env("HSR_SOLO_TRIPS")) > 0) b->solo_trips = (float)atof(env("HSR_SOLO_TRIPS"));
    if (set("HSR_SPLIT")) b->split = atoi(env("HSR_SPLIT")) != 0;
    if (atoi(env("HSR_SPLIT_PERIOD")) > 0) b->split_period = atoi(env("HSR_SPLIT_PERIOD"));
    if (set("HSR_SPLIT_TRIPS") && atof(env("HSR_SPLIT_TRIPS")) >= 0) b->split_trips = (float)atof(env("HSR_SPLIT_TRIPS"));
    if (atoi(env("HSR_SPLIT_MIN_LEFT")) > 0) b->split_min_left = atoi(env("HSR_SPLIT_MIN_LEFT"));
    if (set("HSR_SPLIT_LONE")) b->split_lone = atoi(env("HSR_SPLIT_LONE")) != 0;
    if (atof(env("HSR_SPLIT_LONE_TRIPS")) > 0) b->split_lone_trips = (float)atof(env("HSR_SPLIT_LONE_TRIPS"));
    if (set("HSR_QUEUE")) b->queue = atoi(env("HSR_QUEUE")) != 0;
    if (atoi(env("HSR_QUEUE_CHUNK")) > 0) b->queue_chunk = atoi(env("HSR_QUEUE_CHUNK"));
    b->queue_chunk_set = atoi(env("HSR_QUEUE_CHUNK")) > 0;
    if (set("HSR_MPR_WARM")) b->mpr_warm = atoi(env("HSR_MPR_WARM")) != 0;
    b->schedule = !is0("HSR_SCHEDULE");
    if (atoi(env("HSR_NARROW_BLOCKS")) > 0) b->narrow_blocks = atoi(env("HSR_NARROW_BLOCKS"));
    if (atoi(env("HSR_PPW")) > 0) b->pairs_per_wave = atoi(env("HSR_PPW"));
}
// ... 135 lines not shown
    DevModel &d = b->dm;
    const int G = b->group;
    auto layout = [&](auto g, bool tg) {
        return PersistLayout<decltype(g)::value>(d.njmax, b->ds.kstride, d.npair_pad, d.nlink, d.ngeom, d.nstatic_geom, tg);
    };
    d.nfb = trailing_free_bodies(b, m);
    int row = cfg_const_row(b, m, d);
    if (row >= 0 && kKin3Checks[row].i) {
        const int *lf = m->i32("link_free"), *dl = m->i32("dof_link");
        int nrd = 0;
        for (int k = 0; k < d.nv; k++) nrd += lf[dl[k]] ? 0 : 1;
        const int stage = 12 * d.nv + ((nrd + 3) & ~3) * nrd;
        const int region = by_group(G, [&](auto g) { return layout(g, false).oCnt; });
        if (stage > region) row = -1;
    }
    b->const_row = row;
    b->kin3 = row >= 0 && kKin3Checks[row].i;
    const int rc = stage_hulls(b, m);
    if (rc) return rc;
    auto lds_total = [&](bool tg) { return (size_t)sizeof(float) * by_group(G, [&](auto g) { return layout(g, tg).total; }); };
    const PersistInstance *in_lds = find_instance(row, G, d.nv, false), *in_global = find_instance(row, G, d.nv, true);
    hipFuncAttributes fa;
    b->persist_tg = in_lds && in_global && !b->sw.tables_lds
                    && hipFuncGetAttributes(&fa, (const void *)in_lds->fn) == hipSuccess && lds_total(false) + fa.sharedSizeBytes > 20480
                    && hipFuncGetAttributes(&fa, (const void *)in_global->fn) == hipSuccess && lds_total(true) + fa.sharedSizeBytes <= 20480;
    b->persist_lds_bytes = lds_total(b->persist_tg);
    const PersistInstance *inst = b->persist_tg ? in_global : in_lds;
    if (!fits_persist(b, m) || !inst) { d.nfb = 0; return HSR_OK; }
    b->kernel = inst->fn;
    b->kernel_sv = inst->sv;
    b->split_inst = inst->split;
    b->persist = true;
    for (persist_fn f : {b->kernel, b->kernel_sv})
        if (f && b->persist_lds_bytes > 48 * 1024) HIPCHK(hipFuncSetAttribute((const void *)f, hipFuncAttributeMaxDynamicSharedMemorySize, (int)b->persist_lds_bytes));
    int pb = -1;
    hipDeviceProp_t prop;
    if (hipOccupancyMaxActiveBlocksPerMultiprocessor(&pb, b->kernel, 64, b->persist_lds_bytes) == hipSuccess && pb > 0
        && hipGetDeviceProperties(&prop, b->device) == hipSuccess) b->slots = pb * prop.multiProcessorCount;
    if (b->sw.debug && hipFuncGetAttributes(&fa, (const void *)b->kernel) == hipSuccess)
        fprintf(stderr, "[hsrsim] k_env_step_mf<%d>: regs %d, static LDS %zu, dyn LDS %zu, scratch %zu -> %d workgroups per CU\n", G, fa.numRegs, fa.sharedSizeBytes, b->persist_lds_bytes, fa.localSizeBytes, pb);
    return HSR_OK;
}

static int upload_model(hsr_batch *b, const hsr_model *m) {
    DevModel &d = b->dm;
    const int *sz = m->sizes;
    d.nq = sz[HSR_NQ]; d.nv = sz[HSR_NV]; d.nu = sz[HSR_NU]; d.nlink = sz[HSR_NLINK]; d.nbody = sz[HSR_NBODY];
    d.ngeom = sz[HSR_NGEOM]; d.npair = sz[HSR_NPAIR]; d.nslot = sz[HSR_NSLOT]; d.nconmax = sz[HSR_NCONMAX]; d.njmax = sz[HSR_NJMAX];
    if (d.npair > 384) return fail(HSR_EINVAL, "more than 384 candidate geom pairs");
    if (d.ngeom > 255) return fail(HSR_EINVAL, "more than 255 geoms");
    d.nM = d.nv * (d.nv + 1) / 2;
    d.ndense = sz[13];
    d.timestep = (float)m->opt[0]; d.impratio = (float)m->opt[1]; d.gravz = (float)m->opt[2]; d.tolerance = (float)m->opt[3];
    d.iterations = (int)m->opt[4]; d.ls_iterations = (int)m->opt[5]; d.ls_tolerance = (float)m->opt[6];
    d.mpr_tolerance = (float)m->opt[7]; d.mpr_iterations = (int)m->opt[8]; d.meaninertia = (float)m->opt[9];
    int rc = 0;
#define UI(f) if ((rc = upload_i(b, &d.f, m, #f))) { return rc; }
#define UF(f) if ((rc = upload_f(b, &d.f, m, #f))) { return rc; }
    UI(link_parent) UI(link_dofadr) UI(link_dofnum) UI(link_qposadr) UI(link_free)
    UF(link_pos) UF(link_mass) UF(link_com) UF(link_inertia) UI(link_dofmask)
    UI(dof_link) UI(dof_type) UI(dof_parent) UI(dof_qposadr) UI(dof_limited)
    UF(dof_axis) UF(dof_pos) UF(dof_damping) UF(dof_invweight0) UF(dof_range) UF(dof_solref) UF(dof_solimp)
    UI(body_link) UI(body_mocap) UF(body_pos)
    UI(geom_type) UI(geom_link) UI(geom_meshadr) UI(geom_meshnum)
    UF(geom_pos) UF(geom_size) UF(geom_rbound) UF(geom_invweight) UF(mesh_vert) UF(geom_aabb)
    UI(pair_geom1) UI(pair_geom2) UI(pair_fn) UI(pair_condim) UI(pair_slot)
    UF(pair_friction) UF(pair_solref) UF(pair_solimp)
    UI(act_dof) UF(act_gear) UF(act_kp) UF(act_ctrlrange) UF(act_forcerange)
#undef UI
#undef UF
    return HSR_OK;
}
static int derive_pair_rec(hsr_batch *b, const hsr_model *m) {
    DevModel &d = b->dm;
    const int *g1 = m->i32("pair_geom1"), *g2 = m->i32("pair_geom2"), *cd = m->i32("pair_condim"), *gl = m->i32("geom_link"), *ad = m->i32("act_dof");
    const double *fr = m->f64("pair_friction"), *sr = m->f64("pair_solref"), *si = m->f64("pair_solimp"), *iw = m->f64("geom_invweight");
    std::vector<float> rec((size_t)std::max(d.npair, 1) * 16, 0.f);
    for (int p = 0; p < d.npair; p++) {
        float *r = rec.data() + 16 * p;
        r[0] = (float)cd[p]; r[1] = (float)gl[g1[p]]; r[2] = (float)gl[g2[p]]; r[3] = (float)(iw[2 * g1[p]] + iw[2 * g2[p]]);
        for (int j = 0; j < 5; j++) r[4 + j] = (float)fr[5 * p + j];
        const double dmax = std::min(std::max(si[5 * p + 1], (double)HSR_MINIMP), (double)HSR_MAXIMP), tc = sr[2 * p], dr = sr[2 * p + 1];
        r[9] = (float)(2.0 / (dmax * tc)); r[10] = (float)(1.0 / (dmax * dmax * tc * tc * dr * dr));
        for (int j = 0; j < 5; j++) r[11 + j] = (float)si[5 * p + j];
    }
    std::vector<int> da(std::max(d.nv, 1), -1);
    for (int a = 0; a < d.nu; a++) da[ad[a]] = a;
    const int rc = upload(b, &d.pair_rec, rec);
    return rc ? rc : upload(b, &d.dof_act, da);
}
static int derive_collision_recs(hsr_batch *b, const hsr_model *m) {
    DevModel &d = b->dm;
    const int *g1 = m->i32("pair_geom1"), *g2 = m->i32("pair_geom2"), *fn = m->i32("pair_fn"), *sl = m->i32("pair_slot");
    const int *gl = m->i32("geom_link"), *gt = m->i32("geom_type"), *ma = m->i32("geom_meshadr"), *mn = m->i32("geom_meshnum");
    const double *gp = m->f64("geom_pos"), *gq = m->f64("geom_quat"), *gs = m->f64("geom_size"), *gb = m->f64("geom_aabb"), *gr = m->f64("geom_rbound");
    std::vector<float> rec((size_t)std::max(d.npair, 1) * 8, 0.f), grec((size_t)std::max(d.ngeom, 1) * 32, 0.f);
    for (int p = 0; p < d.npair; p++) {
        float *r = rec.data() + 8 * p;
        r[0] = (float)(g1[p] + 256 * (gt[g1[p]] == GEOM_PLANE ? 1 : 0)); r[1] = (float)g2[p]; r[2] = (float)gr[g1[p]]; r[3] = (float)gr[g2[p]];
        r[4] = (float)fn[p]; r[5] = (float)sl[p]; r[6] = (float)(sl[p + 1] - sl[p]); r[7] = (float)gt[g1[p]];
    }
    for (int gg = 0; gg < d.ngeom; gg++) {
        float *o = grec.data() + 32 * gg, lm[9];
        quat2mat_h(gq + 4 * gg, lm);
        o[0] = (float)gl[gg]; o[1] = (float)gt[gg]; o[2] = (float)mn[gg]; o[3] = (float)ma[gg];
        for (int k = 0; k < 3; k++) o[4 + k] = (float)gp[3 * gg + k];
        o[7] = (float)gr[gg];
        for (int k = 0; k < 9; k++) o[8 + k] = lm[k];
        for (int k = 0; k < 3; k++) o[17 + k] = (float)gs[3 * gg + k];
        for (int k = 0; k < 3; k++) { o[20 + k] = (float)gb[6 * gg + k]; o[24 + k] = (float)gb[6 * gg + 3 + k]; }
    }
    const int rc = upload(b, &d.pair_geo, rec);
    return rc ? rc : upload(b, &d.geom_rec, grec);
}
static int derive_tables(hsr_batch *b, const hsr_model *m) {
    DevModel &d = b->dm;
    int rc = 0;
    {
        const int *lp = m->i32("link_parent");
        std::vector<int> dep(std::max(d.nlink, 1), 0);
        d.maxdepth = 0;
        for (int l = 1; l < d.nlink; l++) { dep[l] = dep[lp[l]] + 1; d.maxdepth = std::max(d.maxdepth, dep[l]); }
        if ((rc = upload(b, &d.link_depth, dep))) return rc;
    }
    {
        size_t cnt = 0;
        const double *mv = m->f64("mesh_vert", &cnt);
        const size_t nvt = cnt / 3;
        std::vector<float> v4((nvt + 1) * 4, 0.f);
        for (size_t i = 0; i < nvt; i++) for (int k = 0; k < 3; k++) v4[4 * i + k] = (float)mv[3 * i + k];
        if ((rc = upload(b, &d.mesh_vert4, v4))) return rc;
        const int *mn = m->i32("geom_meshnum");
        for (int g = 0; g < d.ngeom; g++) if (mn[g] > 256) return fail(HSR_EINVAL, "mesh hull with more than 256 vertices");
    }
    {
        const int *gl = m->i32("geom_link");
        d.nstatic_geom = 0;
        while (d.nstatic_geom < d.ngeom && gl[d.nstatic_geom] == 0) d.nstatic_geom++;
    }
    d.npair_pad = (d.npair + 7) & ~7;
    if (d.npair_pad == 0) d.npair_pad = 8;
    if ((rc = derive_pair_rec(b, m)) || (rc = derive_collision_recs(b, m))) return rc;
    if ((rc = upload_mats(b, &d.link_mat, m, "link_quat"))) return rc;
    if ((rc = upload_mats(b, &d.geom_mat, m, "geom_quat"))) return rc;
    if ((rc = upload_mats(b, &d.body_mat, m, "body_quat"))) return rc;
    d.any_damping = 0;
    { size_t cnt; const double *dmp = m->f64("dof_damping", &cnt); for (size_t i = 0; i < cnt; i++) if (dmp[i] > 0) d.any_damping = 1; }
    d.solimp_general = 0;
    for (const char *nm : {"dof_solimp", "pair_solimp"}) {
        size_t cnt; const double *si = m->f64(nm, &cnt);
        for (size_t i = 4; si && i < cnt; i += 5) { const double pw = si[i] < 1 ? 1 : si[i]; if (pw != 1 && pw != 2) d.solimp_general = 1; }
    }
    d.cv_types = 0;
    {
        const int *g1 = m->i32("pair_geom1"), *g2 = m->i32("pair_geom2"), *fn = m->i32("pair_fn"), *gt = m->i32("geom_type");
        for (int p = 0; p < d.npair; p++) if (fn[p] == FN_CONVEX) d.cv_types |= (1 << (gt[g1[p]] & 7)) | (256 << (gt[g2[p]] & 7));
    }
    return HSR_OK;
}
static int alloc_state(hsr_batch *b) {
    const DevModel &d = b->dm;
    DevState &s = b->ds;
    const size_t N = (size_t)b->N;
    int rc = 0;
    s.N = b->N;
    s.npair_sep = std::max(d.npair, 1);
#define DA(field, rows) if ((rc = dalloc(b, &s.field, (size_t)(rows) * N))) return rc;
    DA(qpos, d.nq) DA(qvel, d.nv) DA(ctrl, d.nu) DA(mocap, 3) DA(warm, d.nv) DA(time, 1)
    DA(done, 1) DA(bad, 1) DA(nsteps, 1)
    DA(xpos, 3 * d.nlink) DA(xmat, 9 * d.nlink) DA(lvel, 6 * d.nlink)
    s.kstride = (9 * d.nv + 15 * d.nlink + 15) & ~15;
    DA(kin_aos, s.kstride)
    DA(con, 8 * d.nslot) DA(ncon_pair, d.npair_pad) DA(sepax, 4 * std::max(d.npair, 1)) DA(septick, std::max(d.npair, 1)) DA(tick, 1) DA(pair_list, std::max(d.npair, 1))
    if ((rc = dalloc(b, &s.pair_count, (size_t)d.npair_pad))) return rc;
    if ((rc = dalloc(b, &s.pair_pack, (size_t)((d.npair_pad + 7) & ~7)))) return rc;
    if ((rc = dalloc(b, &s.geom_c, (size_t)8 * std::max(d.ngeom, 1)))) return rc;
    DA(M, d.nM) DA(qacc, d.nv) DA(qacc_smooth, d.nv) DA(qfrc_smooth, d.nv) DA(qfrc_constraint, d.nv)
    DA(ncon, 1) DA(nefc, 1) DA(niter, 1)
#undef DA
    if ((rc = dalloc(b, &s.phase_cyc, 32 + 40 * 8192))) return rc;
    if ((rc = dalloc(b, &s.capstat, 12))) return rc;
    if ((rc = dalloc(b, &s.trips, N))) return rc;
    if ((rc = dalloc(b, &b->d_slot_env, 2 * (N + 64) + 4 * (size_t)SPLIT_MAX_EXTRA))) return rc;
    const size_t tasks = (N + 1) / 2;
    if ((rc = dalloc(b, &s.q_head, QUEUE_ROUNDS))) return rc;
    if ((rc = dalloc(b, &s.q_wpos, QUEUE_ROUNDS))) return rc;
    if ((rc = dalloc(b, &s.q_items, (size_t)QUEUE_ROUNDS * tasks))) return rc;
    if ((rc = dalloc(b, &s.q_err, 1))) return rc;
    s.sq_cap = (int)N + 4096;
    if ((rc = dalloc(b, &s.sq_items, (size_t)s.sq_cap))) return rc;
    if ((rc = dalloc(b, &s.sq_ctl, SPLIT_CTL_WORDS))) return rc;
    s.solo_servers = 0; s.solo_trips_x4 = 14; s.solo_min_left = 40;
    s.split_period = 0; s.split_trips_x4 = 14; s.split_min_left = 40; s.split_lone_x4 = 0;
    s.q_chunk = 0;
    s.slot_env = nullptr;
    return HSR_OK;
}
static int size_solver(hsr_batch *b) {
    const DevModel &d = b->dm;
    b->group = d.nv <= 16 ? 16 : 32;
    if (d.nv > 32 || d.nq > 64 || d.nlink > NLMAX || d.nconmax > b->group || b->ds.kstride > 8 * 4 * b->group)
        return fail(HSR_EINVAL, "model exceeds the lane-group solver (nv <= 32, nlink <= 16, nconmax <= lanes per env)");
    const int total = by_group(b->group, [&](auto g) { return MfLayout<decltype(g)::value>(d.njmax, b->ds.kstride).total; });
    b->mf_lds_bytes = (size_t)total * (64 / b->group) * sizeof(float);
    if (b->mf_lds_bytes > 160 * 1024) return fail(HSR_EINVAL, "model exceeds the LDS budget of the solver");
    if (b->mf_lds_bytes <= 48 * 1024) return HSR_OK;
    const void *fn = by_group(b->group, [](auto g) { return (const void *)k_solve_mf<decltype(g)::value>; });
    HIPCHK(hipFuncSetAttribute(fn, hipFuncAttributeMaxDynamicSharedMemorySize, (int)b->mf_lds_bytes));
    return HSR_OK;
}
static int size_kinematics(hsr_batch *b) {
    const size_t kb = (size_t)64 * (b->ds.kstride + 24 * b->dm.nlink + 1) * sizeof(float);
    if (kb > 160 * 1024) return fail(HSR_EINVAL, "kinematics tile exceeds LDS");
    if (kb > 48 * 1024) HIPCHK(hipFuncSetAttribute((const void *)k_kinematics, hipFuncAttributeMaxDynamicSharedMemorySize, (int)kb));
    return HSR_OK;
}
static int alloc_staging_and_reset(hsr_batch *b, const hsr_model *m) {
    const DevModel &d = b->dm;
    const size_t N = (size_t)b->N;
    int rc = 0;
    b->stage_floats = N * (size_t)(std::max(std::max(std::max(d.nq + d.nv, 25), 7 * d.nslot), std::max(d.nv * d.nv, 9 * d.nlink)) + d.nu + d.nq + d.nv + 4) + 16;
    if ((rc = dalloc(b, &b->d_stage, b->stage_floats))) return rc;
    if ((rc = dalloc(b, &b->d_stage_u8, N))) return rc;
    if ((rc = dalloc(b, &b->d_stage_i32, N))) return rc;
    HIPCHK(hipEventCreate(&b->ev0));
    HIPCHK(hipEventCreate(&b->ev1));
    if ((rc = upload(b, &b->d_qpos0, m->qpos0.data(), (size_t)d.nq))) return rc;
    hipLaunchKernelGGL(k_build_tables, grid1((size_t)std::max(d.ngeom, (d.npair_pad + 7) & ~7)), dim3(256), 0, b->stream, b->dm, b->ds);
    hipLaunchKernelGGL(k_reset, grid1(N), dim3(256), 0, b->stream, b->dm, b->ds, (const uint8_t *)nullptr, (const float *)nullptr,
                       (const float *)b->d_qpos0, (const float *)nullptr, 0);
    HIPCHK(hipStreamSynchronize(b->stream));
    return HSR_OK;
}

static int batch_init(hsr_batch *b, const hsr_model *m) {
    int rc;
    HIPCHK(hipStreamCreateWithFlags(&b->stream, hipStreamNonBlocking));
    if ((rc = upload_model(b, m)) || (rc = derive_tables(b, m)) || (rc = alloc_state(b)) || (rc = size_solver(b))) return rc;
    if ((rc = plan_persist(b, m)) || (rc = size_kinematics(b))) return rc;
    return alloc_staging_and_reset(b, m);
}
extern "C" int hsr_batch_create(const hsr_model *m, int n_envs, int device_id, hsr_batch **out) {
    if (!m || !out || n_envs <= 0) return fail(HSR_EINVAL, "bad arguments to hsr_batch_create");
    int ndev = 0;
    if (hipGetDeviceCount(&ndev) != hipSuccess || ndev <= 0) return fail(HSR_EDEVICE, "no HIP device available%s");
    if (device_id < 0 || device_id >= ndev) return fail(HSR_EINVAL, "device id out of range");
    HIPCHK(hipSetDevice(device_id));
    hsr_batch *b = new hsr_batch();
    b->model = m; b->N = n_envs; b->device = device_id;
    read_switches(b);
    const int rc = batch_init(b, m);
    if (rc) { hsr_batch_destroy(b); return rc; }
    *out = b;
    return HSR_OK;
}

extern "C" void hsr_batch_destroy(hsr_batch *b) {
    if (!b) return;
    hipSetDevice(b->device);
    if (b->stream) hipStreamSynchronize(b->stream);
    for (auto &kv : b->graphs) hipGraphExecDestroy(kv.second);
    snap_release_all(b);
    replay_release_all(b);
    rollout_release_all(b);
    norm_release_all(b);
    plan_release_all(b);
    for (void *p : b->allocs) hipFree(p);
    if (b->d_rimg) hipFree(b->d_rimg);
    if (b->d_cap) hipFree(b->d_cap);
    for (hipEvent_t ev : b->kev) hipEventDestroy(ev);
    for (auto &pr : b->klog) { hipEventDestroy(pr.first); hipEventDestroy(pr.second); }
    if (b->ev0) hipEventDestroy(b->ev0);
    if (b->ev1) hipEventDestroy(b->ev1);
    if (b->stream) hipStreamDestroy(b->stream);
    delete b;
}
```

hsr_env_amd/csrc/model.h:

```cpp
#pragma once
#include <stdint.h>
#include <hip/hip_runtime.h>

enum { DOF_SLIDE = 0, DOF_HINGE = 1, DOF_FREE_LIN = 2, DOF_FREE_ANG = 3 };
enum { GEOM_PLANE = 0, GEOM_SPHERE = 2, GEOM_CYLINDER = 5, GEOM_BOX = 6, GEOM_MESH = 7 };
enum { FN_PLANE_BOX = 0, FN_PLANE_CONVEX = 1, FN_BOX_BOX = 2, FN_CONVEX = 3 };

struct DevModel {
    int nq, nv, nu, nlink, nbody, ngeom, npair, nslot, nconmax, njmax, nM, ndense;
    float timestep, impratio, gravz, tolerance, ls_tolerance, mpr_tolerance, meaninertia;
    int iterations, ls_iterations, mpr_iterations, any_damping;
    int solimp_general;
    int cv_types;
    const int *link_parent, *link_dofadr, *link_dofnum, *link_qposadr, *link_free;
    const float *link_pos, *link_mat, *link_mass, *link_com, *link_inertia;
    const int *link_dofmask, *link_depth;
    int maxdepth;
    const int *dof_link, *dof_type, *dof_parent, *dof_qposadr, *dof_limited;
    const float *dof_axis, *dof_pos, *dof_damping, *dof_invweight0, *dof_range, *dof_solref, *dof_solimp;
    const int *body_link, *body_mocap;
    const float *body_pos, *body_mat;
    const int *geom_type, *geom_link, *geom_meshadr, *geom_meshnum;
    const float *geom_pos, *geom_mat, *geom_size, *geom_rbound, *geom_invweight, *mesh_vert;
    const float *geom_aabb;
    const float4 *mesh_vert4;
    const int *pair_geom1, *pair_geom2, *pair_fn, *pair_condim, *pair_slot;
    const float *pair_friction, *pair_solref, *pair_solimp;
    const int *act_dof, *dof_act;
    const float *pair_rec;
    const float *pair_geo;
    const float *geom_rec;
    int npair_pad;
    int nstatic_geom;
    int nfb;
    const float *act_gear, *act_kp, *act_ctrlrange, *act_forcerange;
    const int *geom_ldsv;
    const int *ldsv_src;
    int nldsv;
};

struct CaptureDesc { float *cap; const int *slot; int every, R; };
struct StepIO { const float *ctrl; float *obs, *reward; uint8_t *done; int32_t *nsteps; const CaptureDesc *cap; };

struct DevState {
    int N;
    float *qpos, *qvel, *ctrl, *mocap, *warm, *time;
    int *done, *bad, *nsteps;
    float *xpos, *xmat;
    float *lvel;
    float *kin_aos;
    int kstride;
    float *con;
    int *ncon_pair;
    int *pair_count, *pair_list;
    float *sepax;
    int npair_sep;
    int *septick, *tick;
    unsigned *pair_pack;
    float *geom_c;
    float *M, *qacc, *qacc_smooth, *qfrc_smooth, *qfrc_constraint;
    int *ncon, *nefc, *niter;
    int ngoal, goal_a[4], goal_b[4];
    float goal_d[4];
    int *slot_env, *trips;
    int q_chunk;
    int *q_head, *q_wpos, *q_items, *q_err;
    int solo_servers, solo_trips_x4, solo_min_left, sq_cap;
    int *sq_items, *sq_ctl;
    int split_period, split_trips_x4, split_min_left;
    int split_lone_x4;
    unsigned long long *capstat;
    unsigned long long *phase_cyc;
};
```

hsr_env_amd/csrc/persist.h:

```cpp
#pragma once
#include "collide.h"
#include "kin2.h"
#include "kin3.h"
#include "solve_mf.h"
#include "split_logic.h"

template <int G> struct PersistLayout {
    int R, MS, oRows, oCnt, oB, envf, oPoly, oKin, oPair, oGeomC, oGeomS, oLinkTab, total;
    __host__ __device__ PersistLayout(int rows, int kstride, int npair_pad, int nlink, int ngeom, int nstatic, bool tables_global = false) {
        R = rows; MS = G + 1;
        int a = 5 * R > kstride ? 5 * R : kstride;
        oRows = 0; oCnt = (a + 3) & ~3;
        a = oCnt + (npair_pad + 3) / 4;
        int b = G * MS > C2_SIZE * G ? G * MS : C2_SIZE * G;
        const int nmov = ngeom - nstatic;
        const int kin_tmp = 24 * nlink + 2 * G + (16 * nmov > 8 * G ? 16 * nmov : 8 * G);
        if (kin_tmp > b) b = kin_tmp;
        oB = (a + 3) & ~3;
        envf = (oB + b + 3) & ~3;
        oPoly = envf * (64 / G);
        oKin = oPoly + 4 * 48;
        oPair = oKin + KIN2_FLOATS * nlink;
        oGeomC = oPair + (tables_global ? 0 : ((npair_pad + 7) & ~7));
        oGeomS = oGeomC + (tables_global ? 0 : 8 * ngeom);
// ... 321 lines not shown
                reach = reach && norm(pt[0] - pt[1]) < s.goal_d[k];
            }
        }
        if (valid && (sub == n_substeps - 1 || reach)) {
            for (int i = c; i < 3 * m.nlink; i += G) s.xpos[(size_t)i * N + e] = poseL[12 * (i / 3) + 9 + i % 3];
            for (int i = c; i < 9 * m.nlink; i += G) s.xmat[(size_t)i * N + e] = poseL[12 * (i / 9) + i % 9];
            for (int i = c; i < 6 * m.nlink; i += G) { const int l = (i % (3 * m.nlink)) / 3; s.lvel[(size_t)i * N + e] = recL[12 * l + (i < 3 * m.nlink ? 0 : 3) + i % 3]; }
        }
        if (io.cap && valid && (!REP || g == 0)) {
            const CaptureDesc cd = *io.cap;
            const int slot = sub % cd.every == 0 ? cd.slot[e] : -1;
            if (slot >= 0) {
                float *f = cd.cap + (size_t)(sub / cd.every) * 12 * m.nlink * cd.R + slot;
                for (int i = c; i < 3 * m.nlink; i += G) f[(size_t)i * cd.R] = poseL[12 * (i / 3) + 9 + i % 3];
                for (int i = c; i < 9 * m.nlink; i += G) f[(size_t)(3 * m.nlink + i) * cd.R] = poseL[12 * (i / 9) + i % 9];
            }
        }
        PHASE_K(31);
        {
            float *gw = qvelL + G;
            const int oGw = (int)(gw - E);
            auto gaddr = [&](int gi, const float *Ei) -> const float * { return gi < nstat ? lds + L.oGeomS + 16 * gi : Ei + oGw + 16 * (gi - nstat); };
            const float *gcc;
            if constexpr (TG) gcc = s.geom_c; else gcc = lds + L.oGeomC;
            float mymove = 0.f;
            if (valid) {
                for (int gm = c; gm < nmov; gm += G) {
                    const GeomPlaceC k2 = gm < G ? gpc : geom_place_consts(m.geom_rec + 32 * (nstat + gm));
                    m3 Rl; v3 pl;
                    pose_load(poseL + 12 * k2.link, Rl, pl);
                    const float4 lv0 = kl4(recL + 12 * k2.link);
                    const v3 lw = mk3(lv0.x, lv0.y, lv0.z), lvo = mk3(lv0.w, recL[12 * k2.link + 4], recL[12 * k2.link + 5]);
                    const v3 vg = lvo + cross(lw, mulmv(Rl, mk3(k2.q1.x, k2.q1.y, k2.q1.z)));
                    const float smove = 1.25f * m.timestep * (norm(vg) + norm(lw) * k2.q1.w) + 1e-7f;
                    geom_place3(k2, Rl, pl, gw + 16 * gm, smove);
                    mymove = fmaxf(mymove, smove);
                }
            }
            acc_move += __int_as_float(gmax<G>(__float_as_int(mymove)));
            const float skin = hook_no_item_list ? 0.f : HSR_SKIN;
            const bool rebuild = skin <= 0.f || !list_ok || wave_any(valid && 2.f * acc_move >= skin);
            for (int p0 = 0; p0 < m.npair_pad / 4; p0 += G) { const int p = p0 + c; if (p < m.npair_pad / 4) reinterpret_cast<int *>(pcnt)[p] = 0; }
            wave_sync();
            PHASE_K(30);
            const float4 *pg4 = reinterpret_cast<const float4 *>(m.pair_geo);
            const unsigned *sPair;
            if constexpr (TG) sPair = s.pair_pack; else sPair = reinterpret_cast<const unsigned *>(lds + L.oPair);
            unsigned short *sCand = reinterpret_cast<unsigned short *>(poly);
            if (rebuild) {
            int ncand = 0;
            nitems = 0;
            int nit_env[EPB];
#pragma unroll
            for (int j = 0; j < EPB; j++) nit_env[j] = 0;
            auto box_round = [&]() {
                const int take = ncand < 64 ? ncand : 64;
                bool pass = false;
                int it = 0;
                if (tid < take) {
                    it = sCand[tid];
                    const float *Ei = lds + (size_t)(it >> 14) * L.envf;
                    const unsigned pk = sPair[it & 0x3fff];
                    const int g1 = pk_g1(pk), g2 = pk_g2(pk);
                    float rb1, rb2;
                    const Geom A = geom_cached3(gaddr(g1, Ei), gcc + 8 * g1, m.mesh_vert4, rb1, ldsv), B = geom_cached3(gaddr(g2, Ei), gcc + 8 * g2, m.mesh_vert4, rb2, ldsv);
                    pass = pair_cull_box_nb(A, B, rb1, rb2, skin);
                }
                PHASE_S(2, 28);
                const unsigned long long lower = (1ull << tid) - 1ull;
                const int ig = it >> 14;
                bool accept = false;
#pragma unroll
                for (int j = 0; j < EPB; j++) {
                    const unsigned long long bj = __ballot(pass && ig == j);
                    if (pass && ig == j) accept = nit_env[j] + __popcll(bj & lower) < 64;
                    nit_env[j] += __popcll(bj);
                }
                const unsigned long long bal = __ballot(accept);
                if (accept) sItems[nitems + __popcll(bal & lower)] = (unsigned short)it;
                nitems += __popcll(bal);
                const int rest = ncand - take;
                unsigned short mv = 0;
                if (tid < rest) mv = sCand[take + tid];
                wave_sync();
                if (tid < rest) sCand[tid] = mv;
                wave_sync();
                ncand = rest;
                PHASE_S(2, 29);
            };
            {
                const int npair8 = (m.npair_pad + 7) & ~7;
                int pb = 0, u = 8, p0 = 0;
                unsigned mybits = 0;
                for (;;) {
                    if (u == 8 && pb < m.npair) {
                        p0 = pb + 8 * c;
                        uint4 k0 = make_uint4(0, 0, 0, 0), k1 = k0;
                        if (p0 < npair8) { k0 = *reinterpret_cast<const uint4 *>(sPair + p0); k1 = *reinterpret_cast<const uint4 *>(sPair + p0 + 4); }
                        const unsigned pk[8] = {k0.x, k0.y, k0.z, k0.w, k1.x, k1.y, k1.z, k1.w};
                        float4 a1[8], a2[8], nn[8];
#pragma unroll
                        for (int q = 0; q < 8; q++) { const float *w1 = gaddr(pk_g1(pk[q]), E), *w2 = gaddr(pk_g2(pk[q]), E); a1[q] = kl4(w1); a2[q] = kl4(w2); nn[q] = kl4(w1 + 12); }
                        mybits = 0;
#pragma unroll
                        for (int q = 0; q < 8; q++) {
                            const float rad = __uint_as_float(pk[q] & 0xffff0000u) + skin;
                            const v3 r = mk3(a2[q].x - a1[q].x, a2[q].y - a1[q].y, a2[q].z - a1[q].z);
                            const float dpl = dot(r, mk3(nn[q].x, nn[q].y, nn[q].z)), dsq = dot(r, r);
                            const bool hit = pk_fn(pk[q]) <= FN_PLANE_CONVEX ? dpl <= rad : dsq <= rad * rad;
                            mybits |= (valid && (!REP || g == 0) && p0 + q < m.npair && hit) ? 1u << q : 0u;
                        }
                        u = 0; pb += 8 * G;
                        PHASE_S(2, 26);
                    }
                    while (u < 8 && ncand < 64) {
                        const bool pass = (mybits >> u) & 1u;
                        const unsigned long long bal = __ballot(pass);
                        if (pass) sCand[ncand + __popcll(bal & ((1ull << tid) - 1ull))] = (unsigned short)((g << 14) | (p0 + u));
                        ncand += __popcll(bal);
                        u++;
                    }
                    PHASE_S(2, 27);
                    const bool more = u < 8 || pb < m.npair;
                    if (ncand >= 64 || (!more && ncand > 0)) { wave_sync(); box_round(); }
                    else if (!more) break;
                }
            }
            wave_sync();
            trunc_mask = 0;
#pragma unroll
            for (int j = 0; j < EPB; j++) if (nit_env[j] > 64) trunc_mask |= 1 << j;
            acc_move = 0.f; list_ok = true;
            }
            if (trunc_mask && ((trunc_mask >> g) & 1) && valid) cap_item++;
            PHASE(19);
            DBGCNT(2, nitems);
            wave_sync();
            for (int ib = 0; ib < nitems; ib += 64) {
                const bool act = ib + tid < nitems;
                const int it = act ? sItems[ib + tid] : 0;
                const int fn = act ? pk_fn(sPair[it & 0x3fff]) : -1;
                auto item_geoms = [&](int item, Geom &A, Geom &B, ContactOut &o, unsigned char *&cntp) {
                    const int ig = item >> 14, p = item & 0x3fff;
                    float *Ei = lds + (size_t)ig * L.envf;
                    const unsigned pk = sPair[p];
                    const float4 pb = pg4[2 * p + 1];
                    float rb;
                    A = geom_cached3(gaddr(pk_g1(pk), Ei), gcc + 8 * pk_g1(pk), m.mesh_vert4, rb, ldsv);
                    B = geom_cached3(gaddr(pk_g2(pk), Ei), gcc + 8 * pk_g2(pk), m.mesh_vert4, rb, ldsv);
                    o.con = s.con + (size_t)sEnv[ig] * m.nslot * 8; o.slot = (int)pb.y; o.maxcnt = (int)pb.z; o.cnt = 0;
                    cntp = reinterpret_cast<unsigned char *>(Ei + L.oCnt) + p;
                };
                PHASE(20);
                if (fn == FN_PLANE_BOX || fn == FN_PLANE_CONVEX) {
                    Geom G1, G2; ContactOut out; unsigned char *cntp;
                    item_geoms(it, G1, G2, out, cntp);
                    if (fn == FN_PLANE_BOX) collide_plane_box(G1, G2, out); else collide_plane_convex(G1, G2, out);
                    *cntp = (unsigned char)out.cnt;
                }
                PHASE(21);
                {
                    constexpr int MW = 8;
                    constexpr int TM1 = ConvexTypes<MT>::first, TM2 = ConvexTypes<MT>::second;
                    const bool cv = fn == FN_CONVEX;
                    float cdx = 0.f, cdy = 0.f, cdz = 0.f, cmg = 0.f;
                    int cfresh = 0;
                    bool need = false;
                    if (cv) {
                        const int p1 = it & 0x3fff, ig1 = it >> 14;
                        float *sx1 = s.sepax + (size_t)(4 * p1) * N + sEnv[ig1];
                        int *stamp1 = s.septick + (size_t)p1 * N + sEnv[ig1];
                        cdx = sx1[0]; cdy = sx1[N]; cdz = sx1[2 * (size_t)N]; cmg = sx1[3 * (size_t)N];
                        const int tick1 = sTick[ig1];
                        cfresh = (*stamp1 == tick1 - 1 || hook_ignore_stamps) ? 1 : 0;
                        need = true;
                        if (cmg >= 0.f && (cdx != 0.f || cdy != 0.f || cdz != 0.f)) {
                            const unsigned pk1 = sPair[p1];
                            const float *Ei1 = lds + (size_t)ig1 * L.envf;
                            const float left = (cfresh ? cmg : 0.f) - (gaddr(pk_g1(pk1), Ei1)[15] + gaddr(pk_g2(pk1), Ei1)[15]);
                            if (left > 0.f) { sx1[3 * (size_t)N] = left; *stamp1 = tick1; need = false; }
                        }
#ifdef HSR_PAIR_HIST
                        atomicAdd(&s.phase_cyc[32 + 40 * 4096 + p1], 1ull);
#endif
                    }
                    const unsigned long long cbal = __ballot(need);
                    if (need) sMpr[__popcll(cbal & ((1ull << tid) - 1ull))] = (unsigned char)tid;
                    const int ncv = __popcll(cbal);
                    wave_sync();
                    PHASE_M(26);
                    for (int r0 = 0; r0 < ncv; r0 += 64 / MW) {
                        const int k = r0 + tid / MW;
                        const int srcl = 4 * (int)sMpr[k < ncv ? k : 0];
                        v3 d = mk3(__int_as_float(__builtin_amdgcn_ds_bpermute(srcl, __float_as_int(cdx))), __int_as_float(__builtin_amdgcn_ds_bpermute(srcl, __float_as_int(cdy))),
                                   __int_as_float(__builtin_amdgcn_ds_bpermute(srcl, __float_as_int(cdz))));
                        const float mg0 = __int_as_float(__builtin_amdgcn_ds_bpermute(srcl, __float_as_int(cmg)));
                        const bool fresh_cache = __builtin_amdgcn_ds_bpermute(srcl, cfresh) != 0;
                        if (k < ncv) {
                            const int it2 = sItems[ib + sMpr[k]];
                            Geom H1, H2; ContactOut o2; unsigned char *cntp;
                            item_geoms(it2, H1, H2, o2, cntp);
                            float *sx = s.sepax + (size_t)(4 * (it2 & 0x3fff)) * N + sEnv[it2 >> 14];
                            int *stampp = s.septick + (size_t)(it2 & 0x3fff) * N + sEnv[it2 >> 14];
                            const int tick_now = sTick[it2 >> 14];
                            float mg = 0.f;
                            int wid[3] = {0, 0, 0};
                            if (mg0 < 0.f) {
                                if (fresh_cache && mpr_warm) { wid[0] = __float_as_int(d.x); wid[1] = __float_as_int(d.y); wid[2] = __float_as_int(d.z); }
                                d = mk3(0, 0, 0);
                            }
                            const bool have = d.x != 0.f || d.y != 0.f || d.z != 0.f;
                            bool still = false;
                            PHASE_M(27);
                            if (have) {
                                const float gap = -dot(support<MW, TM1>(H1, d) - support<MW, TM2>(H2, -d), d);
                                still = gap > 1e-7f;
                                mg = still ? 0.98f * gap : 0.f;
                            }
                            PHASE_M(28);
                            if (!still) {
                                float depth; v3 dir, pos, sep;
                                int nsup = 0;
                                const bool hit = mpr_penetration<MW, TM1, TM2>(H1, H2, m.mpr_tolerance, m.mpr_iterations, depth, dir, pos, sep, nsup, wid);
#ifdef HSR_PHASE_TIMING
                                if ((tid & (MW - 1)) == 0) { atomicAdd(&sDbg[0], nsup); atomicAdd(&sDbg[1], 1); atomicMax(&sDbg[2], nsup); }
#endif
#ifdef HSR_PAIR_HIST
                                if ((tid & (MW - 1)) == 0) atomicAdd(&s.phase_cyc[32 + 40 * 4096 + 512 + (it2 & 0x3fff)], 1ull);
#endif
                                PHASE_M(29);
                                mg = 0.f;
                                if ((tid & (MW - 1)) == 0) {
                                    if (hit) { o2.add(pos, dir, -depth); sep = mk3(0, 0, 0); }
                                    if (hit && wid[0] > 0 && mpr_warm) sep = mk3(__int_as_float(wid[0]), __int_as_float(wid[1]), __int_as_float(wid[2]));
                                    sx[0] = sep.x; sx[N] = sep.y; sx[2 * (size_t)N] = sep.z;
                                }
                                if (hit && wid[0] > 0 && mpr_warm) mg = -1.f;
                            }
                            if ((tid & (MW - 1)) == 0) { sx[3 * (size_t)N] = mg; *stampp = tick_now; }
                            if ((tid & (MW - 1)) == 0) *cntp = (unsigned char)o2.cnt;
                            PHASE_M(30);
                        }
                    }
                }
                PHASE(22);
                {
                    const bool bb = fn == FN_BOX_BOX;
                    const unsigned long long bbal = __ballot(bb);
                    wave_sync();
                    if (bb) sMpr[__popcll(bbal & ((1ull << tid) - 1ull))] = (unsigned char)tid;
                    const int nbb = __popcll(bbal);
                    wave_sync();
                    PHASE_S(3, 26);
                    for (int r0 = 0; r0 < nbb; r0 += 8) {
                        const int k = r0 + tid / 8;
                        if (k < nbb) {
                            Geom G1, G2; ContactOut out; unsigned char *cntp;
                            item_geoms(sItems[ib + sMpr[k]], G1, G2, out, cntp);
                            PHASE_S(3, 27);
                            const int cnt = collide_box_box_w8(G1, G2, out.con, out.slot, out.maxcnt, poly + 24 * (tid / 8), [&](int idx) { (void)idx; if (idx == 28) { PHASE_S(3, 28); } else if (idx == 29) { PHASE_S(3, 29); } else if (idx == 30) { PHASE_S(3, 30); } else { PHASE_S(3, 31); } });
                            if ((tid & 7) == 0) *cntp = (unsigned char)cnt;
                        }
                    }
                }
                PHASE(23);
            }
        }
        __threadfence_block();
        __syncthreads();
        if constexpr (REP) {
            if (g > 0) for (int i = c; i < m.npair_pad / 4; i += G) reinterpret_cast<int *>(pcnt)[i] = reinterpret_cast<const int *>(lds + L.oCnt)[i];
            wave_sync();
        }
        if (dbg_store && valid) for (int p = c; p < m.npair; p += G) s.ncon_pair[(size_t)e * m.npair_pad + p] = pcnt[p];
        PHASE(17);
        float my_q = 0;
        q4 quat0; quat0.w = 1; quat0.x = quat0.y = quat0.z = 0;
        if (isdof) {
            my_q = qposL[my_qadr];
            if (c == my_quat_lane && my_type == DOF_FREE_ANG) { quat0.w = qposL[my_qadr]; quat0.x = qposL[my_qadr + 1]; quat0.y = qposL[my_qadr + 2]; quat0.z = qposL[my_qadr + 3]; }
        }
        wave_sync();
        const int nfb = (EXACT && G == 32) ? m.nfb : 0;
        float *fbK = poly + (size_t)g * 28 * nfb;
        float *lvbuf = rAref;
        const int lvcap = (2 * R) / 6 < 16 ? (2 * R) / 6 : 16;
        {
#define SOLVE_STORE_DIAG dbg_store
#define SOLVE_COUNT_CAPS 1
#define PAIR_CNT8(p) (*reinterpret_cast<const unsigned long long *>(pcnt + (p)))
#define SOLVE_LANE_TABLES 1
#define SOLVE_LIMITS_FROM_MODEL 1
#include "solve_body.inc"
#undef SOLVE_LANE_TABLES
#undef SOLVE_LIMITS_FROM_MODEL
#undef PAIR_CNT8
#undef SOLVE_COUNT_CAPS
#undef SOLVE_STORE_DIAG
            const float v1 = __shfl_down(vnew, 1, G), v2 = __shfl_down(vnew, 2, G);
            wave_sync();
            float *qn = rJv;
            if (valid && isdof) {
                if (my_type == DOF_SLIDE || my_type == DOF_HINGE || my_type == DOF_FREE_LIN) qn[my_qadr] = my_q + h * vnew;
                else if (c == my_quat_lane) {
                    const v3 w = mk3(vnew, v1, v2);
                    const float wn = norm(w), angle = wn * h;
                    q4 q = quat0;
                    if (angle > 0) {
                        const v3 ax = w * (1.0f / wn);
                        float sn, cs;
                        fast_sincos(0.5f * angle, &sn, &cs);
                        q4 qr;
                        qr.w = cs; qr.x = ax.x * sn; qr.y = ax.y * sn; qr.z = ax.z * sn;
                        q = qnormalized(qmul(quat0, qr));
                    }
                    qn[my_qadr] = q.w; qn[my_qadr + 1] = q.x; qn[my_qadr + 2] = q.y; qn[my_qadr + 3] = q.z;
                }
            }
            wave_sync();
            if (valid) {
                if (c < nq) qpos_c = qn[c];
                qvel_c = vnew; warm_c = qacc_c;
                time_e += h; nsteps_e += 1; nsub_run += 1;
                if (bad) bad_acc = 1;
                if (reach) done = true;
            }
            if (wave_any(valid && reach)) list_ok = false;
            trips_acc += newton_trips;
            if (valid && n_substeps - sub <= 100) own_trips += iter;
            if (valid) run_trips += iter;
            wave_sync();
            PHASE(18);
        }
    }
    const bool last_run = sub_stop >= n_substeps;
    {
    int tid_w = tid0;
    asm volatile("" : "+v"(tid_w));
    PERSIST_LANE_VIEW(tid_w)
    const int was_done = in_range ? s.done[e] : 0;
    if (in_range && (fresh || !(was_done != 0 && nsteps_e == 0))) {
        if (c < nq) s.qpos[(size_t)c * N + e] = qpos_c;
        if (isdof) { s.qvel[(size_t)c * N + e] = qvel_c; s.warm[(size_t)c * N + e] = warm_c; }
        const float bsum = gsum<G>((float)bad_acc);
        if (c == 0 && (!REP || g == 0)) {
            if (cap_con) atomicAdd(&s.capstat[0], (unsigned long long)cap_con);
            if (cap_row) atomicAdd(&s.capstat[1], (unsigned long long)cap_row);
            if (cap_item) atomicAdd(&s.capstat[2], (unsigned long long)cap_item);
            atomicAdd(&s.capstat[3], (unsigned long long)nsub_run);
            s.trips[e] = (sub0 <= n_substeps - 100 || first_run) ? own_trips : s.trips[e] + own_trips;
            s.tick[e] = sTick[g];
            s.time[e] = time_e;
            if (bsum > 0) s.bad[e] = 1;
            s.nsteps[e] = (fresh ? 0 : s.nsteps[e]) + nsteps_e;
            if (fresh) s.done[e] = done ? 1 : 0; else if (done) s.done[e] = 1;
        }
    }
    if (in_range && io.ctrl && last_run) {
        if (io.obs) {
            float *o = io.obs + (size_t)e * (nq + nv);
            if (c < nq) o[c] = qpos_c;
            if (isdof) o[nq + c] = qvel_c;
        }
        if (c == 0) {
            if (io.reward) io.reward[e] = done ? 1.f : 0.f;
            if (io.done) io.done[e] = done ? 1 : 0;
            if (io.nsteps) io.nsteps[e] = s.nsteps[e];
            ENV_STAMP(0, e, __builtin_amdgcn_s_memrealtime());
        }
    }
    if constexpr (!SOLO && HAS_SOLO) {
        if (s.q_chunk && s.solo_servers > 0 && !last_run) {
            const bool hard = in_range && !done && n_substeps - sub1 >= s.solo_min_left && 4 * run_trips >= s.solo_trips_x4 * (sub1 - sub0);
            if (wave_any(hard)) {
                __builtin_amdgcn_fence(__ATOMIC_RELEASE, "agent");
                __builtin_amdgcn_wave_barrier();
                if (hard && c == 0) {
                    const int old = __hip_atomic_fetch_sub(&s.sq_ctl[2], 1, __ATOMIC_RELAXED, __HIP_MEMORY_SCOPE_AGENT);
                    if (old > 0) {
                        const int pos = __hip_atomic_fetch_add(&s.sq_ctl[1], 1, __ATOMIC_RELAXED, __HIP_MEMORY_SCOPE_AGENT);
                        s.slot_env[task * EPB + g] = -1;
                        ENV_STAMP(1, e, (unsigned long long)sub1 | (__builtin_amdgcn_s_memrealtime() << 16));
                        __hip_atomic_store(&s.sq_items[pos], e | (sub1 << 20), __ATOMIC_RELEASE, __HIP_MEMORY_SCOPE_AGENT);
                    } else __hip_atomic_fetch_add(&s.sq_ctl[2], 1, __ATOMIC_RELAXED, __HIP_MEMORY_SCOPE_AGENT);
                }
            }
        }
    }
    if constexpr (SPLIT_INST && !SOLO) {
        if (give) {
            __builtin_amdgcn_fence(__ATOMIC_RELEASE, "agent");
            __builtin_amdgcn_wave_barrier();
            if (c == 0 && ((give >> g) & 1u)) {
                const int pos = __hip_atomic_fetch_add(&s.sq_ctl[SPLIT_RESERVED], 1, __ATOMIC_RELAXED, __HIP_MEMORY_SCOPE_AGENT);
                s.slot_env[task * EPB + g] = -1;
                ENV_STAMP(1, e, (unsigned long long)sub_stop | (__builtin_amdgcn_s_memrealtime() << 16));
                if (pos < s.sq_cap) __hip_atomic_store(&s.sq_items[pos], e | (sub_stop << 20), __ATOMIC_RELEASE, __HIP_MEMORY_SCOPE_AGENT);
                else __hip_atomic_store(s.q_err, 1, __ATOMIC_RELAXED, __HIP_MEMORY_SCOPE_AGENT);
            }
            __threadfence_block();
// ... 78 lines not shown
```

hsr_env_amd/csrc/solve_mf.h:

```cpp
#pragma once
#include "solve_g.h"
#include "kin3.h"

enum { C2_POS = 0, C2_L1 = 3, C2_N = 4, C2_L2 = 7, C2_T1 = 8, C2_ADR = 11, C2_T2 = 12, C2_DIM = 15, C2_MU = 16, C2_F0 = 17,
       C2_F2 = 18, C2_F3 = 19, C2_ZONE = 20, C2_DM = 21, C2_K3 = 22, C2_B = 23, C2_FW = 24, C2_KD = 27, C2_TW = 28, C2_SLOT = 30, C2_PAIR = 31,
       C2_GN = 32, C2_U = 38, C2_SIZE = 44, C2_AX = 4, C2_AXS = 4 };
__device__ __forceinline__ float4 lds4(const float *p) { return *reinterpret_cast<const float4 *>(p); }

template <int G> struct MfLayout {
    int R, MS, oRows, oB, oLv, total, envf;
    __host__ __device__ MfLayout(int rows, int kstride) {
        R = rows; MS = G + 1;
        const int a = 5 * R > kstride ? 5 * R : kstride;
        const int b = G * MS > C2_SIZE * G ? G * MS : C2_SIZE * G;
        oRows = 0; oB = (a + 3) & ~3;
        oLv = (oB + b + 3) & ~3;
        total = oLv + 32;
        envf = total;
    }
};

template <int G, int NK = G> __device__ __forceinline__ float chol_solve_mf(const float (&row)[G], float invd, float b, int nv, int c) {
    asm volatile("" : "+v"(c));
    float nlo[G];
#pragma unroll
    for (int k = 0; k < NK; k++) nlo[k] = (k < c) ? -row[k] : 0.f;
    float sacc = b, y = 0.f;
    static_for<0, NK>([&](auto jc) {
        constexpr int j = decltype(jc)::value;
        if (j < nv) {
            const float t = sacc * invd;
            if (c == j) y = t;
            fmac_bcast<G, j, true>(sacc, nlo[j], bc_prepare<G>(t));
        }
    });
    float x = 0.f;
    static_for<0, NK / 2>([&](auto jc) {
        constexpr int j = NK - 1 - 2 * decltype(jc)::value;
        if (j - 1 < nv) {
            float A, B;
            gsum2<G>(nlo[j] * x, nlo[j - 1] * x, A, B);
            const float xj = (j < nv) ? (y + A) * invd : 0.f;
            if (c == j) x = xj;
            const float t = gbcast<G, j>(nlo[j - 1] * xj);
            if (c == j - 1) x = (y + B + t) * invd;
        }
    });
    if constexpr (NK % 2 == 1) {
        if (0 < nv) { const float tot = gsum<G>(nlo[0] * x); if (c == 0) x = (y + tot) * invd; }
    }
    return x;
}

template <int G, int NK = G> __device__ __forceinline__ float chol_back_mf(const float (&row)[G], float invd, float y, int nv, int c) {
    asm volatile("" : "+v"(c));
    float nlo[G];
#pragma unroll
    for (int k = 0; k < NK; k++) nlo[k] = (k < c) ? -row[k] : 0.f;
    float x = 0.f;
    static_for<0, NK / 2>([&](auto jc) {
        constexpr int j = NK - 1 - 2 * decltype(jc)::value;
        if (j - 1 < nv) {
            float A, B;
            gsum2<G>(nlo[j] * x, nlo[j - 1] * x, A, B);
            const float xj = (j < nv) ? (y + A) * invd : 0.f;
            if (c == j) x = xj;
            const float t = gbcast<G, j>(nlo[j - 1] * xj);
            if (c == j - 1) x = (y + B + t) * invd;
        }
    });
    if constexpr (NK % 2 == 1) {
        if (0 < nv) { const float tot = gsum<G>(nlo[0] * x); if (c == 0) x = (y + tot) * invd; }
    }
    return x;
}

template <int G, int NK, int ND> __device__ __forceinline__ float chol_solve_tail(const float (&row)[G], float invd, float b, int c) {
    asm volatile("" : "+v"(c));
    float nlo[ND > 0 ? ND : 1];
#pragma unroll
    for (int k = 0; k < ND; k++) nlo[k] = (k < c && c < ND) ? -row[k] : 0.f;
    float sacc = b, y = 0.f;
    static_for<0, ND>([&](auto jc) {
        constexpr int j = decltype(jc)::value;
        const float t = sacc * invd;
        if (c == j) y = t;
        fmac_bcast<G, j, true>(sacc, nlo[j], bc_prepare<G>(t));
    });
    float x = 0.f;
    if (c >= ND) x = b * invd * invd;
    static_for<0, ND>([&](auto jc) {
        constexpr int j = ND - 1 - decltype(jc)::value;
        const float tot = (ND <= 16) ? gsum<16>(nlo[j] * x) : gsum<G>(nlo[j] * x);
        if (c == j) x = (y + tot) * invd;
    });
    return x;
}

__device__ __forceinline__ unsigned long long pair_cnt8_(const int *p) {
    unsigned long long r = 0;
#pragma unroll
    for (int k = 0; k < 8; k++) r |= (unsigned long long)(p[k] & 0xff) << (8 * k);
    return r;
}

template <int G>
__global__ void __launch_bounds__(64, 2) k_solve_mf(DevModel m, DevState s, int mode, int goal_body, float geofence, int debug) {
    extern __shared__ __align__(16) float lds[];
    constexpr int EPB = 64 / G, NK = G;
    const MfLayout<G> L(m.njmax, s.kstride);
    const int tid = threadIdx.x, g = tid / G, c = tid % G;
    const int e_raw = blockIdx.x * EPB + g;
    const bool valid = e_raw < s.N && !s.done[e_raw < s.N ? e_raw : 0];
    if (!__syncthreads_or(valid)) return;
    const int e = valid ? e_raw : 0;
    const int N = s.N, nv = m.nv, R = L.R, MS = L.MS;
    float *E = lds + (size_t)g * L.total;
    float *rD = E + L.oRows, *rAref = rD + R, *rJar = rAref + R, *rJv = rJar + R, *rDw = rJv + R;
    float *kAng = E + L.oRows, *kLin = kAng + 3 * nv, *kAnc = kAng + 6 * nv, *lk = kAng + 9 * nv;
    float *M = E + L.oB, *con = E + L.oB;
    float *lvbuf = E + L.oLv;
    const int lvcap = 5;
    const bool isdof = c < nv;
    int bad = 0;
    __shared__ int sParent[32], sMask[NLMAX];
    __shared__ float sMass[NLMAX];
    if (tid < nv) sParent[tid] = m.dof_parent[tid];
    if (tid < m.nlink && tid < NLMAX) { sMask[tid] = m.link_dofmask[tid]; sMass[tid] = m.link_mass[tid]; }

    PHASE_T0();
    const int *pair_cnt_ = s.ncon_pair + (size_t)e * m.npair_pad;
    float qvel_c = 0, warm_c = 0, my_q = 0, my_ctrl = 0, damp_c = 0;
    int my_type = -1, my_qadr = 0, my_quat_lane = -1, my_limited = 0, my_act = -1;
    float lim_lo = 0, lim_hi = 0, lim_sr0 = 1, lim_sr1 = 1, lim_iw = 0, lim_si[5] = {0, 0, 0, 0, 0}, lim_B = 0, lim_K = 0;
    float act_p[6] = {0, 0, 0, 0, 0, 0};
    if (isdof) {
        my_type = m.dof_type[c]; my_qadr = m.dof_qposadr[c]; my_limited = m.dof_limited[c]; my_act = m.dof_act[c];
        my_quat_lane = m.link_dofadr[m.dof_link[c]] + 3;
        damp_c = m.dof_damping[c];
        qvel_c = s.qvel[(size_t)c * N + e]; warm_c = s.warm[(size_t)c * N + e];
        lim_lo = m.dof_range[2 * c]; lim_hi = m.dof_range[2 * c + 1]; lim_sr0 = m.dof_solref[2 * c]; lim_sr1 = m.dof_solref[2 * c + 1];
        lim_iw = m.dof_invweight0[c];
#pragma unroll
        for (int j = 0; j < 5; j++) lim_si[j] = m.dof_solimp[5 * c + j];
        { const float dmax = fminf(fmaxf(lim_si[1], HSR_MINIMP), HSR_MAXIMP); lim_B = 2.0f / (dmax * lim_sr0); lim_K = 1.0f / (dmax * dmax * lim_sr0 * lim_sr0 * lim_sr1 * lim_sr1); }
        my_q = s.qpos[(size_t)my_qadr * N + e];
        if (my_act >= 0) {
            my_ctrl = s.ctrl[(size_t)my_act * N + e];
            act_p[0] = m.act_kp[my_act]; act_p[1] = m.act_gear[my_act];
            act_p[2] = m.act_ctrlrange[2 * my_act]; act_p[3] = m.act_ctrlrange[2 * my_act + 1];
            act_p[4] = m.act_forcerange[2 * my_act]; act_p[5] = m.act_forcerange[2 * my_act + 1];
        }
        if (!(fabsf(qvel_c) <= 1e10f) || !(fabsf(my_q) <= 1e10f)) bad = 1;
    }
    {
        const float4 *src = reinterpret_cast<const float4 *>(s.kin_aos + (size_t)e * s.kstride);
        float4 *dst = reinterpret_cast<float4 *>(kAng);
        const int n4 = s.kstride / 4;
        float4 tmp[8];
#pragma unroll
        for (int i = 0; i < 8; i++) { const int idx = c + i * G; tmp[i] = idx < n4 ? src[idx] : make_float4(0, 0, 0, 0); }
#pragma unroll
        for (int i = 0; i < 8; i++) { const int idx = c + i * G; if (idx < n4) dst[idx] = tmp[i]; }
    }
    q4 quat0; quat0.w = 1; quat0.x = quat0.y = quat0.z = 0;
    if (valid && isdof && c == my_quat_lane && my_type == DOF_FREE_ANG) {
        quat0.w = s.qpos[(size_t)my_qadr * N + e]; quat0.x = s.qpos[(size_t)(my_qadr + 1) * N + e];
        quat0.y = s.qpos[(size_t)(my_qadr + 2) * N + e]; quat0.z = s.qpos[(size_t)(my_qadr + 3) * N + e];
    }
    bool reach = false;
    float time0 = 0;
    int nsteps0 = 0;
    if (valid && c == 0) {
        time0 = s.time[e]; nsteps0 = s.nsteps[e];
        if ((goal_body >= 0 || s.ngoal > 0) && mode != 0) {
            const v3 goal = mk3(s.mocap[e], s.mocap[N + e], s.mocap[2 * N + e]);
            View xpos{s.xpos + e, N}, xmat{s.xmat + e, N};
            auto body_point = [&](int body) -> v3 {
                if (m.body_mocap[body]) return goal;
                const int l = m.body_link[body];
                return xpos.get3(l) + mulmv(xmat.getm(l), ld3(m.body_pos, body));
            };
            reach = true;
            if (goal_body >= 0) reach = norm(body_point(goal_body) - goal) < geofence;
            for (int k = 0; k < s.ngoal; k++) reach = reach && norm(body_point(s.goal_a[k]) - body_point(s.goal_b[k])) < s.goal_d[k];
        }
    }
    constexpr int NDK = -1;
    constexpr bool KIN3 = false;
    constexpr bool REP = false;
    using MT = DevModel;
    constexpr bool hook_jv_per_contact = false, hook_majorant = false, hook_dense_chol = false, EXACT_CT = false;
    constexpr int nfb = 0;
    float *fbK = nullptr;
#define SOLVE_STORE_DIAG true
#define PAIR_CNT8(p) pair_cnt8_(pair_cnt_ + (p))
#include "solve_body.inc"
#undef PAIR_CNT8
#undef SOLVE_STORE_DIAG
    const float v1 = __shfl_down(vnew, 1, G), v2 = __shfl_down(vnew, 2, G);
    PHASE(16);
    if (valid && isdof) {
        s.qvel[(size_t)c * N + e] = vnew;
        s.warm[(size_t)c * N + e] = qacc_c;
        if (my_type == DOF_SLIDE || my_type == DOF_HINGE || my_type == DOF_FREE_LIN) s.qpos[(size_t)my_qadr * N + e] = my_q + h * vnew;
    }
    PHASE(17);
    if (valid && isdof) {
        if (my_type == DOF_FREE_ANG && c == my_quat_lane) {
            const v3 w = mk3(vnew, v1, v2);
            const float wn = norm(w), angle = wn * h;
            if (angle > 0) {
                const v3 ax = w * (1.0f / wn);
                float sn, cs;
                fast_sincos(0.5f * angle, &sn, &cs);
                q4 qr;
                qr.w = cs; qr.x = ax.x * sn; qr.y = ax.y * sn; qr.z = ax.z * sn;
                const q4 q = qnormalized(qmul(quat0, qr));
                s.qpos[(size_t)my_qadr * N + e] = q.w; s.qpos[(size_t)(my_qadr + 1) * N + e] = q.x;
                s.qpos[(size_t)(my_qadr + 2) * N + e] = q.y; s.qpos[(size_t)(my_qadr + 3) * N + e] = q.z;
            }
        }
    }
    PHASE(13);
    const float bsum = gsum<G>((float)bad);
    if (valid && c == 0) {
        s.time[e] = time0 + h;
        s.nsteps[e] = nsteps0 + 1;
        if (bsum > 0) s.bad[e] = 1;
        if (reach) s.done[e] = 1;
    }
    PHASE(13);
    PHASE_FLUSH();
}
```

Before: 557,200 env-steps/s.

## Specialize narrowphase dispatch on present pair kinds and hand-write Cholesky forward solve

Adds a per-config bitmask (np_types) of which narrowphase function kinds and plane-convex geom types appear, so the persistent kernel can compile out unused collision branches and specialize plane-convex support functions by geometry type. Separately, the 16-lane Cholesky tail forward substitution is rewritten in inline assembly using DPP row_newbcast fmac so each step is a tight mul/cmp/cndmask/fmac sequence. The aim is to cut branch code, register pressure and instruction count in the collision and solver hot loops. The inline asm relies on row_newbcast DPP semantics and on vcc clobbers being handled correctly.

```diff
diff --git a/hsr_env_amd/csrc/cfg_consts.h b/hsr_env_amd/csrc/cfg_consts.h
--- a/hsr_env_amd/csrc/cfg_consts.h
+++ b/hsr_env_amd/csrc/cfg_consts.h
@@ -25,7 +25,7 @@
 static const float kKin3F_cfg1[] = {(float)0.0, (float)0.0, (float)0.0, (float)-0.46, (float)-0.081, (float)0.0, (float)1.0, (float)0.0, (float)0.0, (float)0.0, (float)1.0, (float)0.0, (float)0.0, (float)0.0, (float)1.0, (float)1.0, (float)0.0, (float)0.0, (float)0.0, (float)1.0, (float)0.0, (float)0.0, (float)0.0, (float)1.0, (float)0.0, (float)0.0, (float)0.0, (float)-0.026226165780202215, (float)0.0033597159715531835, (float)0.3351183143878767, (float)0.0, (float)0.0, (float)0.0, (float)0.0, (float)0.0, (float)0.0, (float)17.93115297082212, (float)18.05290570568451, (float)5.361962854382956, (float)-0.18414327285216073, (float)0.6395772498672245, (float)-0.2890701869118962, (float)0.0, (float)291.3690145854267, (float)1.0, (float)0.0, (float)0.0, (float)0.0, (float)1.0, (float)0.0, (float)0.0, (float)0.0, (float)0.0, (float)0.0, (float)0.0, (float)0.0};
 struct DevModel_cfg1 : DevModel {
     using kin3 = Kin3_cfg1;
-    static constexpr int nq = 2, nv = 2, nu = 2, nlink = 2, nbody = 47, ngeom = 17, npair = 30, nslot = 30, nconmax = 16, njmax = 48, nM = 3, ndense = 0, npair_pad = 32, nstatic_geom = 2, nfb = 0, maxdepth = 1, iterations = 100, ls_iterations = 50, mpr_iterations = 50, any_damping = 1, solimp_general = 0, cv_types = 49248;
+    static constexpr int nq = 2, nv = 2, nu = 2, nlink = 2, nbody = 47, ngeom = 17, npair = 30, nslot = 30, nconmax = 16, njmax = 48, nM = 3, ndense = 0, npair_pad = 32, nstatic_geom = 2, nfb = 0, maxdepth = 1, iterations = 100, ls_iterations = 50, mpr_iterations = 50, any_damping = 1, solimp_general = 0, cv_types = 49248, np_types = 40970;
     static constexpr float timestep = (float)0.002, impratio = (float)2.5, gravz = (float)-9.81, tolerance = (float)1e-08, ls_tolerance = (float)0.01, mpr_tolerance = (float)1e-06, meaninertia = (float)291.3690145854267;
 };
 struct Kin3_cfg2 {
@@ -51,7 +51,7 @@
 static const float kKin3F_cfg2[] = {(float)0.0, (float)0.0, (float)0.0, (float)-0.46, (float)-0.081, (float)0.0, (float)0.0, (float)0.0, (float)0.422, (float)1.0, (float)0.0, (float)0.0, (float)0.0, (float)1.0, (float)0.0, (float)0.0, (float)0.0, (float)1.0, (float)1.0, (float)0.0, (float)0.0, (float)0.0, (float)1.0, (float)0.0, (float)0.0, (float)0.0, (float)1.0, (float)1.0, (float)0.0, (float)0.0, (float)0.0, (float)1.0, (float)0.0, (float)0.0, (float)0.0, (float)1.0, (float)0.0, (float)0.0, (float)0.0, (float)-0.026226165780202215, (float)0.0033597159715531835, (float)0.3351183143878767, (float)0.0, (float)0.0, (float)0.0, (float)0.0, (float)0.0, (float)0.0, (float)0.0, (float)0.0, (float)0.0, (float)17.93115297082212, (float)18.05290570568451, (float)5.361962854382956, (float)-0.18414327285216073, (float)0.6395772498672245, (float)-0.2890701869118962, (float)0.0003046666666666667, (float)0.0009296666666666669, (float)0.0010416666666666669, (float)0.0, (float)0.0, (float)0.0, (float)0.0, (float)291.3690145854267, (float)1.0, (float)1.0, (float)0.0, (float)0.0, (float)0.0, (float)1.0, (float)0.0, (float)1.0, (float)0.0, (float)0.0, (float)0.0, (float)1.0, (float)0.0, (float)0.0, (float)0.0, (float)1.0, (float)1.0, (float)0.0, (float)0.0, (float)0.0, (float)1.0, (float)0.0, (float)0.0, (float)0.0, (float)1.0, (float)0.0, (float)0.0, (float)0.0, (float)0.0, (float)0.0, (float)0.0, (float)0.0, (float)0.0, (float)0.0, (float)0.0, (float)0.0, (float)0.0, (float)0.0, (float)0.0, (float)0.0, (float)0.0, (float)0.0, (float)0.0, (float)0.0, (float)0.0, (float)0.0, (float)0.0, (float)0.0, (float)0.0};
 struct DevModel_cfg2 : DevModel {
     using kin3 = Kin3_cfg2;
-    static constexpr int nq = 9, nv = 8, nu = 2, nlink = 3, nbody = 48, ngeom = 18, npair = 47, nslot = 57, nconmax = 16, njmax = 48, nM = 36, ndense = 0, npair_pad = 48, nstatic_geom = 2, nfb = 1, maxdepth = 1, iterations = 100, ls_iterations = 50, mpr_iterations = 50, any_damping = 1, solimp_general = 0, cv_types = 49248;
+    static constexpr int nq = 9, nv = 8, nu = 2, nlink = 3, nbody = 48, ngeom = 18, npair = 47, nslot = 57, nconmax = 16, njmax = 48, nM = 36, ndense = 0, npair_pad = 48, nstatic_geom = 2, nfb = 1, maxdepth = 1, iterations = 100, ls_iterations = 50, mpr_iterations = 50, any_damping = 1, solimp_general = 0, cv_types = 49248, np_types = 40975;
     static constexpr float timestep = (float)0.002, impratio = (float)2.5, gravz = (float)-9.81, tolerance = (float)1e-08, ls_tolerance = (float)0.01, mpr_tolerance = (float)1e-06, meaninertia = (float)73.21753814635669;
 };
 struct Kin3_cfg3 {
@@ -77,7 +77,7 @@
 static const float kKin3F_cfg3[] = {(float)0.0, (float)0.0, (float)0.0, (float)-0.46, (float)-0.081, (float)0.0, (float)0.0, (float)0.0, (float)0.5, (float)0.141, (float)0.078, (float)0.0, (float)0.005, (float)0.0, (float)0.345, (float)0.02875, (float)0.0245, (float)0.12300000000000001, (float)0.02875, (float)-0.0245, (float)0.12300000000000001, (float)0.0, (float)0.0, (float)0.422, (float)1.0, (float)0.0, (float)0.0, (float)0.0, (float)1.0, (float)0.0, (float)0.0, (float)0.0, (float)1.0, (float)1.0, (float)0.0, (float)0.0, (float)0.0, (float)1.0, (float)0.0, (float)0.0, (float)0.0, (float)1.0, (float)1.0, (float)0.0, (float)0.0, (float)0.0, (float)1.0, (float)0.0, (float)0.0, (float)0.0, (float)1.0, (float)1.0, (float)0.0, (float)0.0, (float)0.0, (float)1.0, (float)0.0, (float)0.0, (float)0.0, (float)1.0, (float)-0.3846153846153848, (float)0.0, (float)0.9230769230769234, (float)0.0, (float)1.0, (float)0.0, (float)-0.9230769230769234, (float)0.0, (float)-0.3846153846153848, (float)-1.0, (float)0.0, (float)0.0, (float)0.0, (float)-1.0, (float)0.0, (float)0.0, (float)0.0, (float)1.0, (float)-1.0, (float)0.0, (float)0.0, (float)0.0, (float)-1.0, (float)0.0, (float)0.0, (float)0.0, (float)1.0, (float)1.0, (float)0.0, (float)0.0, (float)0.0, (float)1.0, (float)0.0, (float)0.0, (float)0.0, (float)1.0, (float)0.0, (float)0.0, (float)0.0, (float)-0.0347552504774637, (float)0.00021983094136669105, (float)0.32107459322514403, (float)0.0860739520361204, (float)0.03730696680027092, (float)-0.048237067089018815, (float)9.217799537819954e-05, (float)0.005378522674296996, (float)0.16866542736039206, (float)-0.0035563457545128956, (float)-4.7945521502316024e-05, (float)0.10077104775564907, (float)0.00852311385996903, (float)0.004977974163455939, (float)0.05882302952465269, (float)0.008341834250917614, (float)-0.005309505504673415, (float)0.05758153613934645, (float)0.0, (float)0.0, (float)0.0, (float)0.0, (float)0.0, (float)0.0, (float)0.0, (float)0.0, (float)0.0, (float)16.250565221699887, (float)15.957245023907413, (float)4.665512029448585, (float)-0.010427084131348163, (float)1.452231512673702, (float)0.008902574260290282, (float)0.022820083057640606, (float)0.009954369124611695, (float)0.018401382356491202, (float)-0.0025433386248086133, (float)-0.0016008468094781338, (float)-0.003139446595221039, (float)0.09299716849489376, (float)0.08975732788794683, (float)0.009232392506510758, (float)1.6681390623358727e-05, (float)-0.000718335940619342, (float)0.0007228876658435388, (float)0.016929615550871812, (float)0.01666906372617751, (float)0.016474889945292476, (float)1.460447612598356e-06, (float)-6.211650900216932e-05, (float)-7.946875319020003e-07, (float)0.04612543712881295, (float)0.04613579905249317, (float)0.04510770854929418, (float)-2.5023825011582902e-05, (float)-0.00010925138184770646, (float)-0.00015737797343488998, (float)0.046089251928950845, (float)0.04609899116723925, (float)0.04510236718567525, (float)2.5455172651502303e-05, (float)-0.00011036966683664154, (float)0.00016320130800520952, (float)0.0003046666666666667, (float)0.0009296666666666669, (float)0.0010416666666666669, (float)0.0, (float)0.0, (float)0.0, (float)0.0, (float)277.8610092915329, (float)4.2251095673594845, (float)6.613989657308645, (float)1.482377430363842, (float)0.6047254681827968, (float)0.5818031706792063, (float)1.0, (float)1.0, (float)0.0, (float)0.0, (float)0.0, (float)1.0, (float)0.0, (float)0.0, (float)0.0, (float)1.0, (float)0.0, (float)-1.0, (float)0.0, (float)0.0, (float)0.0, (float)1.0, (float)1.0, (float)0.0, (float)0.0, (float)-1.0, (float)0.0, (float)0.0, (float)1.0, (float)0.0, (float)0.0, (float)0.0, (float)1.0, (float)0.0, (float)0.0, (float)0.0, (float)1.0, (float)1.0, (float)0.0, (float)0.0, (float)0.0, (float)1.0, (float)0.0, (float)0.0, (float)0.0, (float)1.0, (float)0.0, (float)0.0, (float)0.0, (float)0.0, (float)0.0, (float)0.0, (float)0.0, (float)0.0, (float)0.0, (float)0.0, (float)0.0, (float)0.0, (float)0.0, (float)0.0, (float)0.0, (float)0.0, (float)0.0, (float)0.0, (float)0.0, (float)0.0, (float)0.0, (float)0.0, (float)0.0, (float)0.0, (float)0.0, (float)0.0, (float)0.0, (float)0.0, (float)0.0, (float)0.0, (float)0.0, (float)0.0, (float)0.0, (float)0.0, (float)0.0, (float)0.0, (float)0.0, (float)0.0, (float)0.0};
 struct DevModel_cfg3 : DevModel {
     using kin3 = Kin3_cfg3;
-    static constexpr int nq = 14, nv = 13, nu = 7, nlink = 8, nbody = 48, ngeom = 18, npair = 114, nslot = 124, nconmax = 16, njmax = 48, nM = 91, ndense = 7, npair_pad = 120, nstatic_geom = 2, nfb = 1, maxdepth = 5, iterations = 100, ls_iterations = 50, mpr_iterations = 50, any_damping = 1, solimp_general = 0, cv_types = 49376;
+    static constexpr int nq = 14, nv = 13, nu = 7, nlink = 8, nbody = 48, ngeom = 18, npair = 114, nslot = 124, nconmax = 16, njmax = 48, nM = 91, ndense = 7, npair_pad = 120, nstatic_geom = 2, nfb = 1, maxdepth = 5, iterations = 100, ls_iterations = 50, mpr_iterations = 50, any_damping = 1, solimp_general = 0, cv_types = 49376, np_types = 40975;
     static constexpr float timestep = (float)0.002, impratio = (float)2.5, gravz = (float)-9.81, tolerance = (float)1e-08, ls_tolerance = (float)0.01, mpr_tolerance = (float)1e-06, meaninertia = (float)46.161990948437406;
 };
 struct Kin3_cfg4 {
@@ -103,7 +103,7 @@
 static const float kKin3F_cfg4[] = {(float)0.0, (float)0.0, (float)0.0, (float)-0.46, (float)-0.081, (float)0.0, (float)0.0, (float)0.0, (float)0.5, (float)0.141, (float)0.078, (float)0.0, (float)0.005, (float)0.0, (float)0.345, (float)0.02875, (float)0.0245, (float)0.12300000000000001, (float)0.02875, (float)-0.0245, (float)0.12300000000000001, (float)0.0, (float)-0.12, (float)0.422, (float)0.0, (float)0.0, (float)0.422, (float)0.0, (float)0.12, (float)0.422, (float)1.0, (float)0.0, (float)0.0, (float)0.0, (float)1.0, (float)0.0, (float)0.0, (float)0.0, (float)1.0, (float)1.0, (float)0.0, (float)0.0, (float)0.0, (float)1.0, (float)0.0, (float)0.0, (float)0.0, (float)1.0, (float)1.0, (float)0.0, (float)0.0, (float)0.0, (float)1.0, (float)0.0, (float)0.0, (float)0.0, (float)1.0, (float)1.0, (float)0.0, (float)0.0, (float)0.0, (float)1.0, (float)0.0, (float)0.0, (float)0.0, (float)1.0, (float)-0.3846153846153848, (float)0.0, (float)0.9230769230769234, (float)0.0, (float)1.0, (float)0.0, (float)-0.9230769230769234, (float)0.0, (float)-0.3846153846153848, (float)-1.0, (float)0.0, (float)0.0, (float)0.0, (float)-1.0, (float)0.0, (float)0.0, (float)0.0, (float)1.0, (float)-1.0, (float)0.0, (float)0.0, (float)0.0, (float)-1.0, (float)0.0, (float)0.0, (float)0.0, (float)1.0, (float)1.0, (float)0.0, (float)0.0, (float)0.0, (float)1.0, (float)0.0, (float)0.0, (float)0.0, (float)1.0, (float)1.0, (float)0.0, (float)0.0, (float)0.0, (float)1.0, (float)0.0, (float)0.0, (float)0.0, (float)1.0, (float)1.0, (float)0.0, (float)0.0, (float)0.0, (float)1.0, (float)0.0, (float)0.0, (float)0.0, (float)1.0, (float)0.0, (float)0.0, (float)0.0, (float)-0.0347552504774637, (float)0.00021983094136669105, (float)0.32107459322514403, (float)0.0860739520361204, (float)0.03730696680027092, (float)-0.048237067089018815, (float)9.217799537819954e-05, (float)0.005378522674296996, (float)0.16866542736039206, (float)-0.0035563457545128956, (float)-4.7945521502316024e-05, (float)0.10077104775564907, (float)0.00852311385996903, (float)0.004977974163455939, (float)0.05882302952465269, (float)0.008341834250917614, (float)-0.005309505504673415, (float)0.05758153613934645, (float)0.0, (float)0.0, (float)0.0, (float)0.0, (float)0.0, (float)0.0, (float)0.0, (float)0.0, (float)0.0, (float)0.0, (float)0.0, (float)0.0, (float)0.0, (float)0.0, (float)0.0, (float)16.250565221699887, (float)15.957245023907413, (float)4.665512029448585, (float)-0.010427084131348163, (float)1.452231512673702, (float)0.008902574260290282, (float)0.022820083057640606, (float)0.009954369124611695, (float)0.018401382356491202, (float)-0.0025433386248086133, (float)-0.0016008468094781338, (float)-0.003139446595221039, (float)0.09299716849489376, (float)0.08975732788794683, (float)0.009232392506510758, (float)1.6681390623358727e-05, (float)-0.000718335940619342, (float)0.0007228876658435388, (float)0.016929615550871812, (float)0.01666906372617751, (float)0.016474889945292476, (float)1.460447612598356e-06, (float)-6.211650900216932e-05, (float)-7.946875319020003e-07, (float)0.04612543712881295, (float)0.04613579905249317, (float)0.04510770854929418, (float)-2.5023825011582902e-05, (float)-0.00010925138184770646, (float)-0.00015737797343488998, (float)0.046089251928950845, (float)0.04609899116723925, (float)0.04510236718567525, (float)2.5455172651502303e-05, (float)-0.00011036966683664154, (float)0.00016320130800520952, (float)0.0003046666666666667, (float)0.0009296666666666669, (float)0.0010416666666666669, (float)0.0, (float)0.0, (float)0.0, (float)0.0003046666666666667, (float)0.0009296666666666669, (float)0.0010416666666666669, (float)0.0, (float)0.0, (float)0.0, (float)0.0003046666666666667, (float)0.0009296666666666669, (float)0.0010416666666666669, (float)0.0, (float)0.0, (float)0.0, (float)0.0, (float)277.8610092915329, (float)4.2251095673594845, (float)6.613989657308645, (float)1.482377430363842, (float)0.6047254681827968, (float)0.5818031706792063, (float)1.0, (float)1.0, (float)1.0, (float)1.0, (float)0.0, (float)0.0, (float)0.0, (float)1.0, (float)0.0, (float)0.0, (float)0.0, (float)1.0, (float)0.0, (float)-1.0, (float)0.0, (float)0.0, (float)0.0, (float)1.0, (float)1.0, (float)0.0, (float)0.0, (float)-1.0, (float)0.0, (float)0.0, (float)1.0, (float)0.0, (float)0.0, (float)0.0, (float)1.0, (float)0.0, (float)0.0, (float)0.0, (float)1.0, (float)1.0, (float)0.0, (float)0.0, (float)0.0, (float)1.0, (float)0.0, (float)0.0, (float)0.0, (float)1.0, (float)1.0, (float)0.0, (float)0.0, (float)0.0, (float)1.0, (float)0.0, (float)0.0, (float)0.0, (float)1.0, (float)1.0, (float)0.0, (float)0.0, (float)0.0, (float)1.0, (float)0.0, (float)0.0, (float)0.0, (float)1.0, (float)1.0, (float)0.0, (float)0.0, (float)0.0, (float)1.0, (float)0.0, (float)0.0, (float)0.0, (float)1.0, (float)1.0, (float)0.0, (float)0.0, (float)0.0, (float)1.0, (float)0.0, (float)0.0, (float)0.0, (float)1.0, (float)0.0, (float)0.0, (float)0.0, (float)0.0, (float)0.0, (float)0.0, (float)0.0, (float)0.0, (float)0.0, (float)0.0, (float)0.0, (float)0.0, (float)0.0, (float)0.0, (float)0.0, (float)0.0, (float)0.0, (float)0.0, (float)0.0, (float)0.0, (float)0.0, (float)0.0, (float)0.0, (float)0.0, (float)0.0, (float)0.0, (float)0.0, (float)0.0, (float)0.0, (float)0.0, (float)0.0, (float)0.0, (float)0.0, (float)0.0, (float)0.0, (float)0.0, (float)0.0, (float)0.0, (float)0.0, (float)0.0, (float)0.0, (float)0.0, (float)0.0, (float)0.0, (float)0.0, (float)0.0, (float)0.0, (float)0.0, (float)0.0, (float)0.0, (float)0.0, (float)0.0, (float)0.0, (float)0.0, (float)0.0, (float)0.0, (float)0.0, (float)0.0, (float)0.0, (float)0.0, (float)0.0, (float)0.0, (float)0.0, (float)0.0, (float)0.0, (float)0.0, (float)0.0, (float)0.0, (float)0.0, (float)0.0, (float)0.0, (float)0.0, (float)0.0, (float)0.0, (float)0.0};
 struct DevModel_cfg4 : DevModel {
     using kin3 = Kin3_cfg4;
-    static constexpr int nq = 28, nv = 25, nu = 7, nlink = 10, nbody = 50, ngeom = 20, npair = 151, nslot = 202, nconmax = 32, njmax = 124, nM = 325, ndense = 7, npair_pad = 152, nstatic_geom = 2, nfb = 3, maxdepth = 5, iterations = 100, ls_iterations = 50, mpr_iterations = 50, any_damping = 1, solimp_general = 0, cv_types = 49376;
+    static constexpr int nq = 28, nv = 25, nu = 7, nlink = 10, nbody = 50, ngeom = 20, npair = 151, nslot = 202, nconmax = 32, njmax = 124, nM = 325, ndense = 7, npair_pad = 152, nstatic_geom = 2, nfb = 3, maxdepth = 5, iterations = 100, ls_iterations = 50, mpr_iterations = 50, any_damping = 1, solimp_general = 0, cv_types = 49376, np_types = 40975;
     static constexpr float timestep = (float)0.002, impratio = (float)2.5, gravz = (float)-9.81, tolerance = (float)1e-08, ls_tolerance = (float)0.01, mpr_tolerance = (float)1e-06, meaninertia = (float)24.244417373187453;
 };
 struct Kin3_cupboard {
@@ -129,23 +129,23 @@
 static const float kKin3F_cupboard[] = {(float)0.0, (float)0.0, (float)0.0, (float)-0.1, (float)0.0, (float)0.418, (float)-0.46, (float)-0.081, (float)0.0, (float)0.0, (float)0.0, (float)0.5, (float)0.141, (float)0.078, (float)0.0, (float)0.005, (float)0.0, (float)0.345, (float)0.02875, (float)0.0245, (float)0.12300000000000001, (float)0.02875, (float)-0.0245, (float)0.12300000000000001, (float)1.0, (float)0.0, (float)0.0, (float)0.0, (float)1.0, (float)0.0, (float)0.0, (float)0.0, (float)1.0, (float)1.0, (float)0.0, (float)0.0, (float)0.0, (float)1.0, (float)0.0, (float)0.0, (float)0.0, (float)1.0, (float)1.0, (float)0.0, (float)0.0, (float)0.0, (float)1.0, (float)0.0, (float)0.0, (float)0.0, (float)1.0, (float)1.0, (float)0.0, (float)0.0, (float)0.0, (float)1.0, (float)0.0, (float)0.0, (float)0.0, (float)1.0, (float)1.0, (float)0.0, (float)0.0, (float)0.0, (float)1.0, (float)0.0, (float)0.0, (float)0.0, (float)1.0, (float)-0.3846153846153848, (float)0.0, (float)0.9230769230769234, (float)0.0, (float)1.0, (float)0.0, (float)-0.9230769230769234, (float)0.0, (float)-0.3846153846153848, (float)-1.0, (float)0.0, (float)0.0, (float)0.0, (float)-1.0, (float)0.0, (float)0.0, (float)0.0, (float)1.0, (float)-1.0, (float)0.0, (float)0.0, (float)0.0, (float)-1.0, (float)0.0, (float)0.0, (float)0.0, (float)1.0, (float)0.0, (float)0.0, (float)0.0, (float)0.0, (float)0.0, (float)0.0, (float)-0.0347552504774637, (float)0.00021983094136669105, (float)0.32107459322514403, (float)0.0860739520361204, (float)0.03730696680027092, (float)-0.048237067089018815, (float)9.217799537819954e-05, (float)0.005378522674296996, (float)0.16866542736039206, (float)-0.0035563457545128956, (float)-4.7945521502316024e-05, (float)0.10077104775564907, (float)0.00852311385996903, (float)0.004977974163455939, (float)0.05882302952465269, (float)0.008341834250917614, (float)-0.005309505504673415, (float)0.05758153613934645, (float)0.0, (float)0.0, (float)0.0, (float)0.0, (float)0.0, (float)0.0, (float)0.0003046666666666667, (float)0.0009296666666666669, (float)0.0010416666666666669, (float)0.0, (float)0.0, (float)0.0, (float)16.250565221699887, (float)15.957245023907413, (float)4.665512029448585, (float)-0.010427084131348163, (float)1.452231512673702, (float)0.008902574260290282, (float)0.022820083057640606, (float)0.009954369124611695, (float)0.018401382356491202, (float)-0.0025433386248086133, (float)-0.0016008468094781338, (float)-0.003139446595221039, (float)0.09299716849489376, (float)0.08975732788794683, (float)0.009232392506510758, (float)1.6681390623358727e-05, (float)-0.000718335940619342, (float)0.0007228876658435388, (float)0.016929615550871812, (float)0.01666906372617751, (float)0.016474889945292476, (float)1.460447612598356e-06, (float)-6.211650900216932e-05, (float)-7.946875319020003e-07, (float)0.04612543712881295, (float)0.04613579905249317, (float)0.04510770854929418, (float)-2.5023825011582902e-05, (float)-0.00010925138184770646, (float)-0.00015737797343488998, (float)0.046089251928950845, (float)0.04609899116723925, (float)0.04510236718567525, (float)2.5455172651502303e-05, (float)-0.00011036966683664154, (float)0.00016320130800520952, (float)0.0, (float)1.0, (float)277.8610092915329, (float)4.2251095673594845, (float)6.613989657308645, (float)1.482377430363842, (float)0.6047254681827968, (float)0.5818031706792063, (float)1.0, (float)0.0, (float)0.0, (float)0.0, (float)1.0, (float)0.0, (float)0.0, (float)0.0, (float)1.0, (float)1.0, (float)0.0, (float)0.0, (float)0.0, (float)1.0, (float)0.0, (float)0.0, (float)0.0, (float)1.0, (float)1.0, (float)0.0, (float)0.0, (float)0.0, (float)1.0, (float)0.0, (float)0.0, (float)0.0, (float)1.0, (float)0.0, (float)-1.0, (float)0.0, (float)0.0, (float)0.0, (float)1.0, (float)1.0, (float)0.0, (float)0.0, (float)-1.0, (float)0.0, (float)0.0, (float)0.0, (float)0.0, (float)0.0, (float)0.0, (float)0.0, (float)0.0, (float)0.0, (float)0.0, (float)0.0, (float)0.0, (float)0.0, (float)0.0, (float)0.0, (float)0.0, (float)0.0, (float)0.0, (float)0.0, (float)0.0, (float)0.0, (float)0.0, (float)0.0, (float)0.0, (float)0.0, (float)0.0, (float)0.0, (float)0.0, (float)0.0, (float)0.0, (float)0.0, (float)0.0, (float)0.0, (float)0.0, (float)0.0, (float)0.0, (float)0.0, (float)0.0, (float)0.0, (float)0.0, (float)0.0};
 struct DevModel_cupboard : DevModel {
     using kin3 = Kin3_cupboard;
-    static constexpr int nq = 14, nv = 13, nu = 7, nlink = 8, nbody = 53, ngeom = 28, npair = 274, nslot = 354, nconmax = 16, njmax = 48, nM = 91, ndense = 13, npair_pad = 280, nstatic_geom = 12, nfb = 0, maxdepth = 5, iterations = 100, ls_iterations = 50, mpr_iterations = 50, any_damping = 1, solimp_general = 0, cv_types = 49376;
+    static constexpr int nq = 14, nv = 13, nu = 7, nlink = 8, nbody = 53, ngeom = 28, npair = 274, nslot = 354, nconmax = 16, njmax = 48, nM = 91, ndense = 13, npair_pad = 280, nstatic_geom = 12, nfb = 0, maxdepth = 5, iterations = 100, ls_iterations = 50, mpr_iterations = 50, any_damping = 1, solimp_general = 0, cv_types = 49376, np_types = 40975;
     static constexpr float timestep = (float)0.002, impratio = (float)2.5, gravz = (float)-9.81, tolerance = (float)1e-08, ls_tolerance = (float)0.01, mpr_tolerance = (float)1e-06, meaninertia = (float)46.161990948437406;
 };
 
-struct CfgConstRow { const char *name; int i[22]; float f[7]; };
+struct CfgConstRow { const char *name; int i[23]; float f[7]; };
 static const CfgConstRow kCfgConsts[] = {
-    {"cfg1", {2, 2, 2, 2, 47, 17, 30, 30, 16, 48, 3, 0, 32, 2, 0, 1, 100, 50, 50, 1, 0, 49248}, {(float)0.002, (float)2.5, (float)-9.81, (float)1e-08, (float)0.01, (float)1e-06, (float)291.3690145854267}},
-    {"cfg2", {9, 8, 2, 3, 48, 18, 47, 57, 16, 48, 36, 0, 48, 2, 1, 1, 100, 50, 50, 1, 0, 49248}, {(float)0.002, (float)2.5, (float)-9.81, (float)1e-08, (float)0.01, (float)1e-06, (float)73.21753814635669}},
-    {"cfg3", {14, 13, 7, 8, 48, 18, 114, 124, 16, 48, 91, 7, 120, 2, 1, 5, 100, 50, 50, 1, 0, 49376}, {(float)0.002, (float)2.5, (float)-9.81, (float)1e-08, (float)0.01, (float)1e-06, (float)46.161990948437406}},
-    {"cfg4", {28, 25, 7, 10, 50, 20, 151, 202, 32, 124, 325, 7, 152, 2, 3, 5, 100, 50, 50, 1, 0, 49376}, {(float)0.002, (float)2.5, (float)-9.81, (float)1e-08, (float)0.01, (float)1e-06, (float)24.244417373187453}},
-    {"cupboard", {14, 13, 7, 8, 53, 28, 274, 354, 16, 48, 91, 13, 280, 12, 0, 5, 100, 50, 50, 1, 0, 49376}, {(float)0.002, (float)2.5, (float)-9.81, (float)1e-08, (float)0.01, (float)1e-06, (float)46.161990948437406}},
+    {"cfg1", {2, 2, 2, 2, 47, 17, 30, 30, 16, 48, 3, 0, 32, 2, 0, 1, 100, 50, 50, 1, 0, 49248, 40970}, {(float)0.002, (float)2.5, (float)-9.81, (float)1e-08, (float)0.01, (float)1e-06, (float)291.3690145854267}},
+    {"cfg2", {9, 8, 2, 3, 48, 18, 47, 57, 16, 48, 36, 0, 48, 2, 1, 1, 100, 50, 50, 1, 0, 49248, 40975}, {(float)0.002, (float)2.5, (float)-9.81, (float)1e-08, (float)0.01, (float)1e-06, (float)73.21753814635669}},
+    {"cfg3", {14, 13, 7, 8, 48, 18, 114, 124, 16, 48, 91, 7, 120, 2, 1, 5, 100, 50, 50, 1, 0, 49376, 40975}, {(float)0.002, (float)2.5, (float)-9.81, (float)1e-08, (float)0.01, (float)1e-06, (float)46.161990948437406}},
+    {"cfg4", {28, 25, 7, 10, 50, 20, 151, 202, 32, 124, 325, 7, 152, 2, 3, 5, 100, 50, 50, 1, 0, 49376, 40975}, {(float)0.002, (float)2.5, (float)-9.81, (float)1e-08, (float)0.01, (float)1e-06, (float)24.244417373187453}},
+    {"cupboard", {14, 13, 7, 8, 53, 28, 274, 354, 16, 48, 91, 13, 280, 12, 0, 5, 100, 50, 50, 1, 0, 49376, 40975}, {(float)0.002, (float)2.5, (float)-9.81, (float)1e-08, (float)0.01, (float)1e-06, (float)46.161990948437406}},
 };
 struct Kin3Check { const int *i; int ni; const float *f; int nf; };
 static const Kin3Check kKin3Checks[] = {{kKin3I_cfg1, (int)(sizeof kKin3I_cfg1 / sizeof(int)), kKin3F_cfg1, (int)(sizeof kKin3F_cfg1 / sizeof(float))}, {kKin3I_cfg2, (int)(sizeof kKin3I_cfg2 / sizeof(int)), kKin3F_cfg2, (int)(sizeof kKin3F_cfg2 / sizeof(float))}, {kKin3I_cfg3, (int)(sizeof kKin3I_cfg3 / sizeof(int)), kKin3F_cfg3, (int)(sizeof kKin3F_cfg3 / sizeof(float))}, {kKin3I_cfg4, (int)(sizeof kKin3I_cfg4 / sizeof(int)), kKin3F_cfg4, (int)(sizeof kKin3F_cfg4 / sizeof(float))}, {kKin3I_cupboard, (int)(sizeof kKin3I_cupboard / sizeof(int)), kKin3F_cupboard, (int)(sizeof kKin3F_cupboard / sizeof(float))}};
 static inline void cfg_const_values(const DevModel &d, int *i, float *f) {
-    const int iv[] = {d.nq, d.nv, d.nu, d.nlink, d.nbody, d.ngeom, d.npair, d.nslot, d.nconmax, d.njmax, d.nM, d.ndense, d.npair_pad, d.nstatic_geom, d.nfb, d.maxdepth, d.iterations, d.ls_iterations, d.mpr_iterations, d.any_damping, d.solimp_general, d.cv_types};
+    const int iv[] = {d.nq, d.nv, d.nu, d.nlink, d.nbody, d.ngeom, d.npair, d.nslot, d.nconmax, d.njmax, d.nM, d.ndense, d.npair_pad, d.nstatic_geom, d.nfb, d.maxdepth, d.iterations, d.ls_iterations, d.mpr_iterations, d.any_damping, d.solimp_general, d.cv_types, d.np_types};
     const float fv[] = {d.timestep, d.impratio, d.gravz, d.tolerance, d.ls_tolerance, d.mpr_tolerance, d.meaninertia};
-    for (int k = 0; k < 22; k++) i[k] = iv[k];
+    for (int k = 0; k < 23; k++) i[k] = iv[k];
     for (int k = 0; k < 7; k++) f[k] = fv[k];
 }
diff --git a/hsr_env_amd/csrc/collide.h b/hsr_env_amd/csrc/collide.h
--- a/hsr_env_amd/csrc/collide.h
+++ b/hsr_env_amd/csrc/collide.h
@@ -229,6 +229,13 @@
 }
 template <class T, class = void> struct ConvexTypes { static constexpr int first = GEOM_TYPES_ANY, second = GEOM_TYPES_ANY; };
 template <class T> struct ConvexTypes<T, std::enable_if_t<!std::is_same<T, DevModel>::value>> { static constexpr int first = T::cv_types & 0xff, second = (T::cv_types >> 8) & 0xff; };
+enum { FN_KINDS_ANY = 0xf };
+template <class T, class = void> struct NarrowTypes { static constexpr int kinds = FN_KINDS_ANY, plane_convex = GEOM_TYPES_ANY; };
+template <class T> struct NarrowTypes<T, std::enable_if_t<!std::is_same<T, DevModel>::value>> { static constexpr int kinds = T::np_types & 0xf, plane_convex = (T::np_types >> 8) & 0xff; };
+template <int FK, int F> __device__ __forceinline__ bool fn_kind_is(int fn) {
+    if constexpr (((FK >> F) & 1) == 0) return false;
+    else return fn == F;
+}
 template <int W = 1, int TM = GEOM_TYPES_ANY> __device__ __forceinline__ v3 support(const Geom &G, v3 dir, int *vid = nullptr) {
     const v3 dl = mulmtv(G.mat, dir);
     v3 loc;
@@ -319,9 +326,9 @@
     }
 }
 
-__device__ __forceinline__ void collide_plane_convex(const Geom &P, const Geom &Cx, ContactOut &out) {
+template <int TM = GEOM_TYPES_ANY> __device__ __forceinline__ void collide_plane_convex(const Geom &P, const Geom &Cx, ContactOut &out) {
     const v3 n = col(P.mat, 2);
-    const v3 p = support(Cx, -n);
+    const v3 p = support<1, TM>(Cx, -n);
     const float dist = dot(p - P.pos, n);
     if (!(dist < 0)) return;
     out.add(p - n * (0.5f * dist), n, dist);
@@ -336,7 +343,7 @@
 #pragma unroll
     for (int i = 0; i < 3; i++) {
         if (nk >= out.maxcnt) break;
-        const v3 q = support(Cx, (t1 * cs[i][0] + t2 * cs[i][1]) * 0.1f - n);
+        const v3 q = support<1, TM>(Cx, (t1 * cs[i][0] + t2 * cs[i][1]) * 0.1f - n);
         const float dq = dot(q - P.pos, n);
         bool take = dq < 0;
 #pragma unroll
diff --git a/hsr_env_amd/csrc/host_create.h b/hsr_env_amd/csrc/host_create.h
--- a/hsr_env_amd/csrc/host_create.h
+++ b/hsr_env_amd/csrc/host_create.h
@@ -311,9 +311,14 @@
         for (size_t i = 4; si && i < cnt; i += 5) { const double pw = si[i] < 1 ? 1 : si[i]; if (pw != 1 && pw != 2) d.solimp_general = 1; }
     }
     d.cv_types = 0;
+    d.np_types = 0;
     {
         const int *g1 = m->i32("pair_geom1"), *g2 = m->i32("pair_geom2"), *fn = m->i32("pair_fn"), *gt = m->i32("geom_type");
-        for (int p = 0; p < d.npair; p++) if (fn[p] == FN_CONVEX) d.cv_types |= (1 << (gt[g1[p]] & 7)) | (256 << (gt[g2[p]] & 7));
+        for (int p = 0; p < d.npair; p++) {
+            if (fn[p] == FN_CONVEX) d.cv_types |= (1 << (gt[g1[p]] & 7)) | (256 << (gt[g2[p]] & 7));
+            d.np_types |= 1 << (fn[p] & 3);
+            if (fn[p] == FN_PLANE_CONVEX) d.np_types |= 256 << (gt[g2[p]] & 7);
+        }
     }
     return HSR_OK;
 }
diff --git a/hsr_env_amd/csrc/model.h b/hsr_env_amd/csrc/model.h
--- a/hsr_env_amd/csrc/model.h
+++ b/hsr_env_amd/csrc/model.h
@@ -12,6 +12,7 @@
     int iterations, ls_iterations, mpr_iterations, any_damping;
     int solimp_general;
     int cv_types;
+    int np_types;
     const int *link_parent, *link_dofadr, *link_dofnum, *link_qposadr, *link_free;
     const float *link_pos, *link_mat, *link_mass, *link_com, *link_inertia;
     const int *link_dofmask, *link_depth;
diff --git a/hsr_env_amd/csrc/persist.h b/hsr_env_amd/csrc/persist.h
--- a/hsr_env_amd/csrc/persist.h
+++ b/hsr_env_amd/csrc/persist.h
@@ -497,17 +497,18 @@
                     cntp = reinterpret_cast<unsigned char *>(Ei + L.oCnt) + p;
                 };
                 PHASE(20);
-                if (fn == FN_PLANE_BOX || fn == FN_PLANE_CONVEX) {
+                constexpr int FK = NarrowTypes<MT>::kinds;
+                if (fn_kind_is<FK, FN_PLANE_BOX>(fn) || fn_kind_is<FK, FN_PLANE_CONVEX>(fn)) {
                     Geom G1, G2; ContactOut out; unsigned char *cntp;
                     item_geoms(it, G1, G2, out, cntp);
-                    if (fn == FN_PLANE_BOX) collide_plane_box(G1, G2, out); else collide_plane_convex(G1, G2, out);
+                    if (fn_kind_is<FK, FN_PLANE_BOX>(fn)) collide_plane_box(G1, G2, out); else collide_plane_convex<NarrowTypes<MT>::plane_convex>(G1, G2, out);
                     *cntp = (unsigned char)out.cnt;
                 }
                 PHASE(21);
                 {
                     constexpr int MW = 8;
                     constexpr int TM1 = ConvexTypes<MT>::first, TM2 = ConvexTypes<MT>::second;
-                    const bool cv = fn == FN_CONVEX;
+                    const bool cv = fn_kind_is<FK, FN_CONVEX>(fn);
                     float cdx = 0.f, cdy = 0.f, cdz = 0.f, cmg = 0.f;
                     int cfresh = 0;
                     bool need = false;
@@ -590,7 +591,7 @@
                 }
                 PHASE(22);
                 {
-                    const bool bb = fn == FN_BOX_BOX;
+                    const bool bb = fn_kind_is<FK, FN_BOX_BOX>(fn);
                     const unsigned long long bbal = __ballot(bb);
                     wave_sync();
                     if (bb) sMpr[__popcll(bbal & ((1ull << tid) - 1ull))] = (unsigned char)tid;
diff --git a/hsr_env_amd/csrc/solve_mf.h b/hsr_env_amd/csrc/solve_mf.h
--- a/hsr_env_amd/csrc/solve_mf.h
+++ b/hsr_env_amd/csrc/solve_mf.h
@@ -75,12 +75,38 @@
     return x;
 }
 
+#define HSR_FWD_STEP_(J, NL) "v_mul_f32 %[t], %[sacc], %[invd]\n\tv_cmp_eq_u32 vcc, " #J ", %[c]\n\tv_cndmask_b32 %[y], %[y], %[t], vcc\n\t" \
+                             "v_fmac_f32_dpp %[sacc], %[t], %[" #NL "] row_newbcast:" #J " row_mask:0xf bank_mask:0xf\n\t"
+#define HSR_FWD_LAST_(J) "v_mul_f32 %[t], %[sacc], %[invd]\n\tv_cmp_eq_u32 vcc, " #J ", %[c]\n\tv_cndmask_b32 %[y], %[y], %[t], vcc"
+template <int J, bool LAST> __device__ __forceinline__ void solve_step16_fwd(float &sacc, float &y, float &t, float invd, float nl, int c) {
+    if constexpr (!LAST)
+        asm volatile("v_mul_f32 %[t], %[sacc], %[invd]\n\tv_cmp_eq_u32 vcc, %[j], %[c]\n\tv_cndmask_b32 %[y], %[y], %[t], vcc\n\t"
+                     "v_fmac_f32_dpp %[sacc], %[t], %[nl] row_newbcast:%[j] row_mask:0xf bank_mask:0xf"
+                     : [sacc] "+v"(sacc), [y] "+v"(y), [t] "=&v"(t) : [invd] "v"(invd), [nl] "v"(nl), [c] "v"(c), [j] "n"(J) : "vcc");
+    else
+        asm volatile("v_mul_f32 %[t], %[sacc], %[invd]\n\tv_cmp_eq_u32 vcc, %[j], %[c]\n\tv_cndmask_b32 %[y], %[y], %[t], vcc"
+                     : [y] "+v"(y), [t] "=&v"(t) : [sacc] "v"(sacc), [invd] "v"(invd), [c] "v"(c), [j] "n"(J) : "vcc");
+}
+template <int ND> __device__ __forceinline__ void solve_fwd16(float sacc, float &y, float invd, const float (&nlo)[ND > 0 ? ND : 1], int c) {
+    float t;
+    if constexpr (ND == 7)
+        asm volatile(HSR_FWD_STEP_(0, n0) HSR_FWD_STEP_(1, n1) HSR_FWD_STEP_(2, n2) HSR_FWD_STEP_(3, n3) HSR_FWD_STEP_(4, n4) HSR_FWD_STEP_(5, n5) HSR_FWD_LAST_(6)
+                     : [sacc] "+v"(sacc), [y] "+v"(y), [t] "=&v"(t)
+                     : [invd] "v"(invd), [c] "v"(c), [n0] "v"(nlo[0]), [n1] "v"(nlo[1]), [n2] "v"(nlo[2]), [n3] "v"(nlo[3]), [n4] "v"(nlo[4]), [n5] "v"(nlo[5]) : "vcc");
+    else
+        static_for<0, ND>([&](auto jc) { constexpr int j = decltype(jc)::value; solve_step16_fwd<j, j == ND - 1>(sacc, y, t, invd, nlo[j], c); });
+}
+#undef HSR_FWD_STEP_
+#undef HSR_FWD_LAST_
 template <int G, int NK, int ND> __device__ __forceinline__ float chol_solve_tail(const float (&row)[G], float invd, float b, int c) {
     asm volatile("" : "+v"(c));
     float nlo[ND > 0 ? ND : 1];
 #pragma unroll
     for (int k = 0; k < ND; k++) nlo[k] = (k < c && c < ND) ? -row[k] : 0.f;
     float sacc = b, y = 0.f;
+    if constexpr (G == 16 && ND > 0) {
+        solve_fwd16<ND>(sacc, y, invd, nlo, c);
+    } else
     static_for<0, ND>([&](auto jc) {
         constexpr int j = decltype(jc)::value;
         const float t = sacc * invd;
```

New measurement: 557,100 env-steps/s. No clear change (-0.0%).
